# harskish/fluctus

Measured on AMD Instinct MI355X. Metric: Mrays/s (primary+shadow) at 1080p, 8 bounces, higher is better.
Workload: dtype f32; 1 GPU; kitchen-proc (procedural stand-in for Country Kitchen OBJ), 1920x1080, 8 bounces, env-map MIS under night.hdr, separate material queues; width=1920, height=1080, max_bounces=8, triangles=495648, bvh=sbvh, bvh_nodes=342315, num_tasks_per_gpu=16777216, num_tasks_whole_job=16777216, scaling_mode=weak: --num-tasks paths in flight per rank, wavefronts_per_gpu=1, fused_logic_materials=True, fused_bsdf_set=1, ext_order=2, refill_extend=8208, overlap=2, regroup=1

## Files before the change

fluctus_amd/csrc/api.hip:

```cpp
#include "flx_ctx.h"
#include <cstring>
#include <cstdlib>

thread_local std::string flxd::g_create_error;

static uint32_t localPixels(const flx_ctx *c)
{
    uint32_t npix = c->params.width * c->params.height;
    if (npix <= c->fr.rank) return 1;
    return (npix - c->fr.rank + c->fr.nranks - 1) / c->fr.nranks;
}

static int allocMoments(flx_ctx *c)
{
    freeAll(c->momAllocs);
    c->fr.moments = nullptr;
    if (!c->moments || !c->fr.localPixels) return 0;
    const size_t n = (size_t)c->fr.localPixels * 4;
    HIPCHK(c, dalloc(c, c->momAllocs, &c->fr.moments, n) ? hipErrorOutOfMemory : hipSuccess);
    HIPCHK(c, hipMemsetAsync(c->fr.moments, 0, n * 4, c->stream));
    return 0;
}
static int allocAov(flx_ctx *c)
{
    c->dn.release();
    freeAll(c->aovAllocs);
    c->fr.aovAlbedo = c->fr.aovNormal = c->fr.aovAlbedoOut = c->fr.aovNormalOut = nullptr;
    if (!c->denoiser || !c->fr.localPixels) return 0;
    const size_t n = (size_t)c->fr.localPixels * 4;
    float *buf[4] = {nullptr, nullptr, nullptr, nullptr};
    for (int i = 0; i < 4; i++) {
        HIPCHK(c, dalloc(c, c->aovAllocs, &buf[i], n) ? hipErrorOutOfMemory : hipSuccess);
        HIPCHK(c, hipMemsetAsync(buf[i], 0, n * 4, c->stream));
    }
    c->fr.aovAlbedo = buf[0]; c->fr.aovNormal = buf[1]; c->fr.aovAlbedoOut = buf[2]; c->fr.aovNormalOut = buf[3];
    return 0;
}

static int allocFrame(flx_ctx *c)
{
    uint32_t lp = localPixels(c);
    if (lp == c->fr.localPixels && c->fr.pixels) return 0;
    HIPCHK(c, hipStreamSynchronize(c->stream));
    c->releaseFrameFeatures();
    freeAll(c->frameAllocs);
    HIPCHK(c, dalloc(c, c->frameAllocs, &c->fr.pixels, (size_t)lp * 4) ? hipErrorOutOfMemory : hipSuccess);
    HIPCHK(c, dalloc(c, c->frameAllocs, &c->fr.preview, (size_t)lp * 4) ? hipErrorOutOfMemory : hipSuccess);
    HIPCHK(c, hipMemsetAsync(c->fr.pixels, 0, (size_t)lp * 16, c->stream));
    HIPCHK(c, hipMemsetAsync(c->fr.preview, 0, (size_t)lp * 16, c->stream));
    c->fr.localPixels = lp;
    if (allocMoments(c)) return 1;
    return allocAov(c);
}

static bool refill_value_ok(int v) { return v == 0 || (v > 0 && (v & 0xFF) >= 1 && (v & 0xFF) <= 64 && (v >> 8) <= 64); }

void flxd::pickSchedule(flx_ctx *c)
{
    c->overlap = c->overlapOpt >= 0 ? c->overlapOpt : 2;
    c->refillShadow = c->refillShadowOpt >= 0 ? c->refillShadowOpt : 0;
}

static int optionBuffers(flx_ctx *c, bool split, bool regen)
{
    HIPCHK(c, hipSetDevice(c->device));
    if (split && !c->splitRecA) {
        uint32_t *cnt = nullptr; uint4 *a = nullptr, *b = nullptr;
        if (dalloc(c, c->fixedAllocs, &cnt, shadow_split_count_words()) || dalloc(c, c->fixedAllocs, &a, (size_t)c->splitCapA * shadow_split_lists() * 4) ||
            dalloc(c, c->fixedAllocs, &b, (size_t)c->splitCapB * shadow_split_lists() * 4)) { c->err = "flx_set_option(shadow_split): out of device memory for the continuation records"; return 1; }
        HIPCHK(c, hipMemsetAsync(cnt, 0, (size_t)shadow_split_count_words() * 4, c->stream));
        c->splitCounts = cnt; c->splitRecA = a; c->splitRecB = b;
    }
    if (regen && !c->lookback) {
        unsigned long long *lb = nullptr;
        if (dalloc(c, c->fixedAllocs, &lb, (size_t)logic_lookback_words(c->numTasks))) { c->err = "flx_set_option(regen): out of device memory for the look-back words"; return 1; }
        HIPCHK(c, hipMemsetAsync(lb, 0, (size_t)logic_lookback_words(c->numTasks) * 8, c->stream));
        c->lookback = lb;
    }
    return 0;
}

extern "C" {

const char *flx_last_error(flx_ctx *c) { return c ? c->err.c_str() : g_create_error.c_str(); }

int flx_create(int device, uint32_t num_tasks, flx_ctx **out)
{
    *out = nullptr;
    int ndev = 0;
    hipError_t e = hipGetDeviceCount(&ndev);
    if (e != hipSuccess || ndev <= 0) { g_create_error = "flx_create: no HIP device available (libfluctus_hip.so has no CPU fallback)"; return 1; }
    if (device < 0 || device >= ndev) { g_create_error = "flx_create: bad device index"; return 1; }
    if (num_tasks == 0) { g_create_error = "flx_create: num_tasks must be > 0"; return 1; }
    flx_ctx *c = new flx_ctx();
    c->device = device; c->numTasks = num_tasks;
#ifdef FLX_LAB
    if (const char *e = getenv("FLX_REFILL_EXTEND")) { const int v = atoi(e); if (refill_value_ok(v)) c->refillExt = v; }
    if (const char *e = getenv("FLX_REFILL_SHADOW")) { const int v = atoi(e); if (v < 0 || refill_value_ok(v)) { c->refillShadowOpt = v; c->refillShadow = v < 0 ? 0 : v; } }
#endif
    auto fail = [&](const char *what, hipError_t err) { g_create_error = std::string(what) + ": " + hipGetErrorString(err); flx_destroy(c); return 1; };
    if ((e = hipSetDevice(device)) != hipSuccess) return fail("hipSetDevice", e);
#ifndef FLX_STREAM_PRIO
#define FLX_STREAM_PRIO 0
#endif
    {
        int least = 0, greatest = 0;
        (void)hipDeviceGetStreamPriorityRange(&least, &greatest);
        const int pMain = FLX_STREAM_PRIO ? greatest : 0, pSecond = FLX_STREAM_PRIO ? least : 0;
        if ((e = hipStreamCreateWithPriority(&c->stream, hipStreamNonBlocking, pMain)) != hipSuccess) return fail("hipStreamCreate", e);
        if ((e = hipStreamCreateWithPriority(&c->stream2, hipStreamNonBlocking, pSecond)) != hipSuccess) return fail("hipStreamCreate", e);
    }
    if ((e = hipEventCreateWithFlags(&c->evPreExt, hipEventDisableTiming)) != hipSuccess || (e = hipEventCreateWithFlags(&c->evShadow, hipEventDisableTiming)) != hipSuccess ||
        (e = hipEventCreateWithFlags(&c->evPostLogic, hipEventDisableTiming)) != hipSuccess) return fail("hipEventCreate", e);
    const size_t N = num_tasks;
    c->st.numTasks = num_tasks;
    for (int r = 0; r < S_NUM_REC; r++) {
        if (dalloc(c, c->fixedAllocs, &c->st.rec[r], N)) return fail("hipMalloc(state)", hipErrorOutOfMemory);
        (void)hipMemsetAsync(c->st.rec[r], 0, N * sizeof(float4), c->stream);
    }
    if (dalloc(c, c->fixedAllocs, &c->st.phase, N) || dalloc(c, c->fixedAllocs, &c->mkStats, 4)) return fail("hipMalloc(state)", hipErrorOutOfMemory);
    (void)hipMemsetAsync(c->st.phase, 0, N * 4, c->stream); (void)hipMemsetAsync(c->mkStats, 0, 16, c->stream);
    if (dalloc(c, c->fixedAllocs, &c->st.blocked, N) || dalloc(c, c->fixedAllocs, &c->st.pickProb, N) || dalloc(c, c->fixedAllocs, &c->st.firstDiffuse, N))
        return fail("hipMalloc(state)", hipErrorOutOfMemory);
    (void)hipMemsetAsync(c->st.blocked, 0, N * 4, c->stream); (void)hipMemsetAsync(c->st.pickProb, 0, N * 4, c->stream); (void)hipMemsetAsync(c->st.firstDiffuse, 0, N * 4, c->stream);
    for (int q = 0; q < FLX_NUM_QUEUES; q++) {
        if (dalloc(c, c->fixedAllocs, &c->qs.q[q], N)) return fail("hipMalloc(queue)", hipErrorOutOfMemory);
        (void)hipMemsetAsync(c->qs.q[q], 0, N * 4, c->stream);
    }
    if (dalloc(c, c->fixedAllocs, &c->qs.counters, 8) || dalloc(c, c->fixedAllocs, &c->qs.cursors, FLX_NUM_BLOCK_CURSORS * FLX_CURSOR_STRIDE)) return fail("hipMalloc(counters)", hipErrorOutOfMemory);
    (void)hipMemsetAsync(c->qs.counters, 0, 32, c->stream);
    (void)hipMemsetAsync(c->qs.cursors, 0, 4 * FLX_NUM_BLOCK_CURSORS * FLX_CURSOR_STRIDE, c->stream);
    const size_t auxStride = logic_aux_stride(num_tasks);
    const size_t queueAuxWords = logic_queue_aux_words(num_tasks);
    if (dalloc(c, c->fixedAllocs, &c->member, N) || dalloc(c, c->fixedAllocs, &c->blockCounts, (size_t)7 * auxStride) || dalloc(c, c->fixedAllocs, &c->queueAux, queueAuxWords))
        return fail("hipMalloc(logic aux)", hipErrorOutOfMemory);
    if (dalloc(c, c->fixedAllocs, &c->logicError, 1)) return fail("hipMalloc(logic error flag)", hipErrorOutOfMemory);
    (void)hipMemsetAsync(c->logicError, 0, 4, c->stream);
    (void)hipMemsetAsync(c->blockCounts, 0, (size_t)7 * auxStride * 4, c->stream);
    (void)hipMemsetAsync(c->queueAux, 0, queueAuxWords * 4, c->stream);
    { hipDeviceProp_t prop; if (hipGetDeviceProperties(&prop, device) == hipSuccess && prop.multiProcessorCount > 0) c->numCUs = prop.multiProcessorCount; }
    if (dalloc(c, c->fixedAllocs, &c->stats, FLX_NUM_TRACE_STATS)) return fail("hipMalloc(stats)", hipErrorOutOfMemory);
    (void)hipMemsetAsync(c->stats, 0, FLX_NUM_TRACE_STATS * 8, c->stream);
#ifdef FLX_LAB_RSTATS
    flxd::g_lab_rstats = c->stats;
#endif
    c->splitCapA = ((num_tasks / 2 / shadow_split_lists()) + 64u) & ~63u; c->splitCapB = ((num_tasks / 8 / shadow_split_lists()) + 64u) & ~63u;
    if (dalloc(c, c->fixedAllocs, &c->totals, 8)) return fail("hipMalloc(totals)", hipErrorOutOfMemory);
    (void)hipMemsetAsync(c->totals, 0, 64, c->stream);
    if (dalloc(c, c->fixedAllocs, &c->fr.currPixelIdx, 1)) return fail("hipMalloc(cursor)", hipErrorOutOfMemory);
    (void)hipMemsetAsync(c->fr.currPixelIdx, 0, 4, c->stream);
    c->fr.rank = 0; c->fr.nranks = 1; c->fr.localPixels = 0;
    if ((e = hipHostMalloc((void **)&c->pinned, sizeof(flx_queue_counters) * c->pinnedSlots)) != hipSuccess) return fail("hipHostMalloc", e);
    if ((e = hipHostMalloc((void **)&c->pinnedIdx, sizeof(uint32_t) * c->pinnedSlots)) != hipSuccess) return fail("hipHostMalloc", e);
    if ((e = hipHostMalloc((void **)&c->pinnedMk, 16 * c->pinnedSlots)) != hipSuccess) return fail("hipHostMalloc", e);
    {
        float4 *rgba; float2 *rec; float *pdf;
        if (dalloc(c, c->envAllocs, &rgba, 1) || dalloc(c, c->envAllocs, &rec, 1) || dalloc(c, c->envAllocs, &pdf, 1))
            return fail("hipMalloc(env)", hipErrorOutOfMemory);
        const float one = 1.0f; const float2 rec1 = make_float2(1.0f, 0.0f );
        (void)hipMemsetAsync(rgba, 0, 16, c->stream);
        (void)hipMemcpy(rec, &rec1, 8, hipMemcpyHostToDevice); (void)hipMemcpy(pdf, &one, 4, hipMemcpyHostToDevice);
        c->sc.envRGBA = rgba; c->sc.aliasRec = rec; c->sc.pdfTable = pdf; c->sc.envW = c->sc.envH = 1;
        float4 *nee; if (dalloc(c, c->envAllocs, &nee, 2)) return fail("hipMalloc(env)", hipErrorOutOfMemory);
        launch_env_nee_table(c->stream, c->sc, nee, 1u); c->sc.neeRec = nee;
    }
    if ((e = hipStreamSynchronize(c->stream)) != hipSuccess) return fail("hipStreamSynchronize", e);
    *out = c;
    return 0;
}

int flx_destroy(flx_ctx *c)
{
    if (!c) return 0;
    c->phase = PH_IDLE;
    (void)hipSetDevice(c->device);
    if (c->stream) (void)hipStreamSynchronize(c->stream);
    if (c->comm) { flx_group_destroy(c); }
    c->releaseFrameFeatures(); c->gather.release(); c->ob.release(); c->ml.releaseBuffers();
    freeAll(c->sceneAllocs); freeAll(c->spillAllocs); freeAll(c->envAllocs); freeAll(c->frameAllocs); freeAll(c->aovAllocs); freeAll(c->momAllocs); freeAll(c->fixedAllocs);
    if (c->pinned) (void)hipHostFree(c->pinned);
    if (c->pinnedIdx) (void)hipHostFree(c->pinnedIdx);
    if (c->pinnedMk) (void)hipHostFree(c->pinnedMk);
    for (auto &ev : c->events) { (void)hipEventDestroy(ev.a); (void)hipEventDestroy(ev.b); }
    for (auto e : c->eventPool) (void)hipEventDestroy(e);
    if (c->stream2) { (void)hipStreamSynchronize(c->stream2); (void)hipStreamDestroy(c->stream2); }
    if (c->evPreExt) (void)hipEventDestroy(c->evPreExt);
    if (c->evShadow) (void)hipEventDestroy(c->evShadow);
    if (c->evPostLogic) (void)hipEventDestroy(c->evPostLogic);
    if (c->stream) (void)hipStreamDestroy(c->stream);
    delete c;
    return 0;
}

uint32_t flx_num_tasks(flx_ctx *c) { return c->numTasks; }
void *flx_stream(flx_ctx *c) { (void)enter(c, CALL_PEEK); return (void *)c->stream; }

int flx_set_params(flx_ctx *c, const void *p240)
{
    ENTER(c, CALL_OBSERVE);
    NEED(c, p240, "flx_set_params: null");
    HIPCHK(c, hipSetDevice(c->device));
    const uint32_t oldW = c->params.width, oldH = c->params.height;
    memcpy(&c->params, p240, sizeof(flx_render_params));
    NEED(c, c->params.width > 0 && c->params.height > 0, "flx_set_params: zero-sized framebuffer");
    if (c->params.width != oldW || c->params.height != oldH) { c->ad.state.dropped(); c->temporal.state.imageResized(); }
    c->haveParams = true;
    return allocFrame(c);
}

int flx_set_partition(flx_ctx *c, uint32_t rank, uint32_t nranks)
{
    ENTER(c, CALL_OBSERVE);
    NEED(c, nranks >= 1 && rank < nranks, "flx_set_partition: bad rank");
    c->fr.rank = rank; c->fr.nranks = nranks;
    c->ad.state.dropped();
    c->temporal.state.partitionSet();
    return c->haveParams ? allocFrame(c) : 0;
}
uint32_t flx_local_pixels(flx_ctx *c) { return c->fr.localPixels; }

int flx_get_counters_async(flx_ctx *c, void *out32)
{
    NEED(c, out32, "flx_get_counters_async: null");
    ENTER(c, CALL_QUIET);
    HIPCHK(c, hipSetDevice(c->device));
    flushExt(c);
    if ((int)c->pending.size() >= c->pinnedSlots) { c->err = "too many outstanding counter reads; call flx_finish"; return 1; }
    int slot = c->nextSlot; c->nextSlot = (c->nextSlot + 1) % c->pinnedSlots;
    HIPCHK(c, hipMemcpyAsync(&c->pinned[slot], c->qs.counters, 32, hipMemcpyDeviceToHost, c->stream));
    c->pending.push_back({out32, slot});
    return 0;
}

int flx_finish(flx_ctx *c)
{
    ENTER(c, CALL_QUIET);
    HIPCHK(c, hipSetDevice(c->device));
    HIPCHK(c, hipStreamSynchronize(c->stream));
    if (c->regenUsed) {
        uint32_t e = 0; HIPCHK(c, hipMemcpy(&e, c->logicError, 4, hipMemcpyDeviceToHost));
        c->regenUsed = false;
        if (e) {
            HIPCHK(c, hipMemset(c->logicError, 0, 4));
            c->err = "k_logic: the in-kernel regeneration's look-back timed out (paths regenerated by that pass are invalid: reset the renderer)"; return 1;
        }
    }
    for (auto &p : c->pending) memcpy(p.user, &c->pinned[p.slot], 32);
    c->pending.clear();
    for (auto &p : c->pendingMk) memcpy(p.first, c->pinnedMk + 4 * p.second, 16);
    c->pendingMk.clear();
    for (auto &ev : c->events) {
        float ms = 0.0f;
        if (hipEventElapsedTime(&ms, ev.a, ev.b) == hipSuccess) { c->kMs[ev.kernel] += ms; c->kLaunches[ev.kernel]++; }
        c->eventPool.push_back(ev.a); c->eventPool.push_back(ev.b);
    }
    c->events.clear();
    return 0;
}

int flx_pixel_index_update(flx_ctx *c, uint32_t npix, uint32_t nnew)
{
    ENTER(c, CALL_NEUTRAL);
    NEED(c, npix > 0, "flx_pixel_index_update: zero pixels");
    HIPCHK(c, hipSetDevice(c->device));
    c->hostPixelIdx = (uint32_t)(((uint64_t)c->hostPixelIdx + nnew) % npix);
    int slot = c->nextIdxSlot; c->nextIdxSlot = (c->nextIdxSlot + 1) % c->pinnedSlots;
    c->pinnedIdx[slot] = c->hostPixelIdx;
    HIPCHK(c, hipMemcpyAsync(c->fr.currPixelIdx, &c->pinnedIdx[slot], 4, hipMemcpyHostToDevice, c->stream));
    return 0;
}
int flx_pixel_index_reset(flx_ctx *c)
{
    ENTER(c, CALL_NEUTRAL);
    HIPCHK(c, hipSetDevice(c->device));
    c->hostPixelIdx = 0;
    HIPCHK(c, hipMemsetAsync(c->fr.currPixelIdx, 0, 4, c->stream));
    return 0;
}

int flx_counter_totals(flx_ctx *c, uint64_t *out8, int reset)
{
    ENTER(c, CALL_QUIET);
    HIPCHK(c, hipSetDevice(c->device));
    HIPCHK(c, hipMemcpyAsync(out8, c->totals, 64, hipMemcpyDeviceToHost, c->stream));
    if (reset) HIPCHK(c, hipMemsetAsync(c->totals, 0, 64, c->stream));
    HIPCHK(c, hipStreamSynchronize(c->stream));
    return 0;
}

int flx_read_pixels(flx_ctx *c, int which, float *out)
{
    ENTER(c, CALL_NEUTRAL);
    NEED(c, c->fr.pixels && out, "flx_read_pixels: no framebuffer");
    HIPCHK(c, hipSetDevice(c->device));
    NEED(c, which >= 0 && which <= 7, "flx_read_pixels: which must be 0..7");
    NEED(c, which != 6 || c->dn.have, "flx_read_pixels: which = 6 is the output of flx_denoise (option \"denoiser\" on): none since the buffers were made");
    NEED(c, which != 7 || c->fr.moments, "flx_read_pixels: which = 7 (the luminance moments) needs flx_set_option(ctx, \"moments\", 1)");
    const float *src[8] = {c->fr.pixels, c->fr.preview, c->fr.aovAlbedoOut, c->fr.aovNormalOut, c->fr.aovAlbedo, c->fr.aovNormal, c->dn.out, c->fr.moments};
    NEED(c, src[which], "flx_read_pixels: the denoiser feature buffers need flx_set_option(ctx, \"denoiser\", 1)");
    HIPCHK(c, hipMemcpyAsync(out, src[which], (size_t)c->fr.localPixels * 16, hipMemcpyDeviceToHost, c->stream));
    HIPCHK(c, hipStreamSynchronize(c->stream));
    return 0;
}
int flx_write_pixels(flx_ctx *c, int which, const float *in)
{
    ENTER(c, CALL_NEUTRAL);
    NEED(c, c->fr.pixels && in, "flx_write_pixels: no framebuffer");
    HIPCHK(c, hipSetDevice(c->device));
    NEED(c, which == 0 || which == 4 || which == 5 || which == 7, "flx_write_pixels: which must be 0, 4 or 5, or 7 with option \"moments\"");
    NEED(c, which != 7 || c->fr.moments, "flx_write_pixels: which = 7 (the luminance moments) needs flx_set_option(ctx, \"moments\", 1)");
    float *dst = which == 0 ? c->fr.pixels : which == 4 ? c->fr.aovAlbedo : which == 5 ? c->fr.aovNormal : c->fr.moments;
    NEED(c, dst, "flx_write_pixels: the denoiser feature buffers need flx_set_option(ctx, \"denoiser\", 1)");
    HIPCHK(c, hipMemcpyAsync(dst, in, (size_t)c->fr.localPixels * 16, hipMemcpyHostToDevice, c->stream));
    HIPCHK(c, hipStreamSynchronize(c->stream));
    return 0;
}
int flx_copy_pixels_to_device(flx_ctx *c, void *dst)
{
    ENTER(c, CALL_OBSERVE);
    NEED(c, c->fr.pixels && dst, "flx_copy_pixels_to_device: no framebuffer");
    HIPCHK(c, hipSetDevice(c->device));
    HIPCHK(c, hipMemcpyAsync(dst, c->fr.pixels, (size_t)c->fr.localPixels * 16, hipMemcpyDeviceToDevice, c->stream));
    return 0;
}

int flx_set_option(flx_ctx *c, const char *name, int value)
{
    ENTER(c, CALL_PEEK);
    if (name && strcmp(name, "xcd_remap") == 0) { c->xcdRemap = value; return 0; }
    if (name && strcmp(name, "fuse") == 0 && (value == 0 || value == 1)) { c->fuse = value; return 0; }
    if (name && strcmp(name, "ext_order") == 0 && value >= 0 && value <= 2) { c->extOrder = value; return 0; }
    if (name && strcmp(name, "regen") == 0 && (value == 0 || value == 1)) { if (value && optionBuffers(c, false, true)) return 1; c->regenOpt = value; return 0; }
    if (name && strcmp(name, "regen_prep") == 0 && (value == 0 || value == 1)) { c->prepOpt = value; return 0; }
    if (name && strcmp(name, "regroup") == 0 && value >= -1 && value <= 1) { c->regroupOpt = value; c->regroup = value >= 0 ? value : c->regroupAuto; return 0; }
    if (name && strcmp(name, "fuse_set") == 0 && (value == 1 || value == 31)) { c->fuseSet = value; return 0; }
    if (name && strcmp(name, "overlap") == 0 && value >= -1 && value <= 2) { ENTER(c, CALL_OBSERVE); c->overlapOpt = value; pickSchedule(c); return 0; }
    if (name && strcmp(name, "shadow_tree") == 0 && (value == 2 || value == 4)) { ENTER(c, CALL_OBSERVE); c->shadowTree = value; return 0; }
    if (name && strcmp(name, "extend_tree") == 0 && (value == 2 || value == 4)) { ENTER(c, CALL_OBSERVE); c->extendTree = value; return 0; }
    if (name && strcmp(name, "denoiser") == 0 && (value == 0 || value == 1)) {
        ENTER(c, CALL_OBSERVE);
        if (c->denoiser != value) { c->denoiser = value; HIPCHK(c, hipSetDevice(c->device)); HIPCHK(c, hipStreamSynchronize(c->stream)); return allocAov(c); }
        return 0;
    }
    if (name && strcmp(name, "moments") == 0 && (value == 0 || value == 1)) {
        ENTER(c, CALL_OBSERVE);
        if (!value) c->ad.state.dropped();
        if (c->moments != value) { c->moments = value; HIPCHK(c, hipSetDevice(c->device)); HIPCHK(c, hipStreamSynchronize(c->stream)); return allocMoments(c); }
        return 0;
    }
    if (name && strcmp(name, "motion_history") == 0 && (value == 0 || value == 1)) {
        ENTER(c, CALL_OBSERVE);
        NEED(c, !value || !c->deformHistory, "flx_set_option: \"motion_history\" cannot be switched on while \"deform_history\" is on (which keeps the history across flx_objects_pose too)");
        if (!value) c->temporal.state.motionHistoryOff();
        c->motionHistory = value;
        return 0;
    }
    if (name && strcmp(name, "deform_history") == 0 && (value == 0 || value == 1)) {
        ENTER(c, CALL_OBSERVE);
        NEED(c, !value || !c->motionHistory, "flx_set_option: \"deform_history\" cannot be switched on while \"motion_history\" is on (switch that off: this option follows a pose too)");
        if (!value) c->temporal.state.deformHistoryOff();
        c->deformHistory = value;
        return 0;
    }
    if (name && strcmp(name, "mesh_lights") == 0 && (value == 0 || value == 1)) {
        ENTER(c, CALL_OBSERVE);
        c->ml.state.optionSet(value != 0);
        return meshLightsSync(c);
    }
    if (name && strcmp(name, "mesh_lights_wavefront") == 0 && (value == 0 || value == 1)) {
        ENTER(c, CALL_OBSERVE);
        c->ml.state.wavefrontSet(value != 0);
        return 0;
    }
    if (name && strcmp(name, "refill_extend") == 0 && refill_value_ok(value)) { ENTER(c, CALL_OBSERVE); c->refillExt = value; return 0; }
    if (name && strcmp(name, "refill_shadow") == 0 && (value == -1 || refill_value_ok(value))) { ENTER(c, CALL_OBSERVE); c->refillShadowOpt = value; pickSchedule(c); return 0; }
    if (name && (strcmp(name, "refill_extend") == 0 || strcmp(name, "refill_shadow") == 0)) { c->err = "flx_set_option: refill value must be 0 or refillMin (1..64) | waitMax (0..64) << 8"; return 1; }
    if (name && strcmp(name, "shadow_split") == 0 && value >= 0 && (value & 0xFF) <= 255 && (value >> 8) <= 255 && ((value & 0xFF) > 0 || value == 0)) { ENTER(c, CALL_OBSERVE); if (value && optionBuffers(c, true, false)) return 1; c->shadowSplit = value; return 0; }
    if (name && strcmp(name, "shadow_split_limit") == 0 && value >= 0) { ENTER(c, CALL_OBSERVE); c->splitLimit = (uint32_t)value; return 0; }
    if (name && strcmp(name, "eager_bump") == 0 && (value == 0 || value == 1)) { c->eagerBump = value; return 0; }
    if (name && strcmp(name, "node_layout") == 0 && (value == 0 || value == 1)) { c->nodeLayout = value; return 0; }
    c->err = std::string("flx_set_option: unknown option ") + (name ? name : "(null)");
    return 1;
}
static int phaseCode(const flx_ctx *c)
{
    return c->phase | (c->rawHits ? 8 : 0) | (c->matQueuesEmpty ? 16 : 0);
}
int flx_get_option(flx_ctx *c, const char *name, int *value)
{
    NEED(c, name && value, "flx_get_option: null");
    const struct { const char *n; int v; } tab[] = {
        {"xcd_remap", c->xcdRemap}, {"fuse", c->fuse}, {"overlap", c->overlap}, {"shadow_tree", c->shadowTree}, {"extend_tree", c->extendTree},
        {"denoiser", c->denoiser}, {"moments", c->moments}, {"motion_history", c->motionHistory}, {"deform_history", c->deformHistory},{"mesh_lights", c->ml.state.on ? 1 : 0}, {"mesh_lights_wavefront", c->ml.state.wavefront ? 1 : 0}, {"eager_bump", c->eagerBump}, {"node_layout", c->nodeLayout}, {"fuse_set", c->fuseSet}, {"ext_order", c->extOrder}, {"regen", c->regenOpt}, {"regroup", c->regroup}, {"regen_prep", c->prepOpt}, {"refill_extend", c->refillExt}, {"refill_shadow", c->refillShadow}, {"shadow_split", c->shadowSplit}, {"fused_queue_mask", (int)fused_queue_mask(fuseSetNow(c))}, {"fuse_set_now", fuseSetNow(c)}};
    for (const auto &t : tab) if (strcmp(name, t.n) == 0) { *value = t.v; return 0; }
    if (strcmp(name, "phase") == 0) { *value = phaseCode(c); return 0; }
    if (strcmp(name, "wide_far") == 0) { *value = wideFar(c); return 0; }
    c->err = std::string("flx_get_option: unknown option ") + name;
    return 1;
}

}
```

fluctus_amd/csrc/api_wavefront.hip:

```cpp
#include "flx_ctx.h"

struct Step { bool launchDeferred, commitRaw; int next; };
static Step transition(int ph, Call call)
{
    const bool deferred = ph == PH_DEFER_LOGIC || ph == PH_DEFER_LOGIC_RAYGEN;
    const bool chain = deferred || ph == PH_CHAIN || ph == PH_CHAIN_EXT;
    switch (call) {
    case CALL_LOGIC:     return {deferred, false, PH_IDLE};
    case CALL_RAYGEN:    if (ph == PH_DEFER_LOGIC) return {false, false, PH_DEFER_LOGIC_RAYGEN};
                         return {deferred, false, chain ? PH_CHAIN : PH_IDLE};
    case CALL_MATERIALS: if (deferred) return {false, false, PH_CHAIN};
                         return {false, true, chain ? PH_CHAIN : PH_IDLE};
    case CALL_EXTEND:    return {deferred, true, chain ? PH_CHAIN_EXT : PH_EXT};
    case CALL_SHADOW:    return {deferred, false, PH_IDLE};
    case CALL_QUIET:     return {deferred, false, deferred ? PH_CHAIN : ph};
    case CALL_NEUTRAL:   return {deferred, false, PH_IDLE};
    case CALL_PEEK:      return {deferred, true, deferred ? PH_CHAIN : ph};
    case CALL_OBSERVE:   return {deferred, true, PH_IDLE};
    }
    return {deferred, true, PH_IDLE};
}
void flxd::flushExt(flx_ctx *c) { if (c->qs.extPend) { launch_bump_extension(c->stream, c->qs.counters, c->qs.extPend); c->qs.extPend = 0; } }
static void flushExtIfPending(flx_ctx *c, uint32_t bits) { if (c->qs.extPend & bits) flushExt(c); }
static int runRaygen(flx_ctx *c, int appendExt = 1, bool alreadyDone = false, bool prepared = false)
{
    flushExtIfPending(c, 1u << FLX_Q_RAYGEN);
    if (!alreadyDone) { ScopedTimer t(c, FLX_K_RAYGEN); launch_raygen(c->stream, c->st, c->qs, c->fr, c->params, appendExt, prepared ? 1 : 0); }
    c->qs.extPend |= 1u << FLX_Q_RAYGEN;
    if (c->eagerBump) flushExt(c);
    LAUNCHED(c);
    return 0;
}
static int materialise(flx_ctx *c)
{
    if (!c->rawHits) return 0;
    c->rawHits = false;
    HIPCHK(c, hipSetDevice(c->device));
    launch_materialise(c->stream, c->st, c->sc, c->params, (uint32_t)c->numCUs);
    LAUNCHED(c);
    return 0;
}
static int extOrderFor(const flx_ctx *c, int fused, int raygenFirst) { return !fused ? 0 : (c->extOrder == 2 && (!raygenFirst || !c->raygenQueueEmpty)) ? 1 : c->extOrder; }
int flxd::fuseSetNow(const flx_ctx *c) { return c->params.wfSeparateQueues ? c->fuseSet : 31; }
static int runLogic(flx_ctx *c, int first, int fused, int raygenFirst)
{
    const int raw = (c->rawHits && fused != 0 && raygenFirst && !first) ? 1 : 0;
    if (!raw && materialise(c)) return 1;
    c->rawHits = false;
    flushExt(c);
#ifdef FLX_LAB_NOJOIN
    if (c->labIter >= 2) HIPCHK(c, hipStreamWaitEvent(c->stream, c->evLab[c->labIter & 1u], 0));
#endif
    const int order = extOrderFor(c, fused, raygenFirst);
    const int regen = (raw && c->regenOpt && c->lookback && logic_can_regenerate() && c->raygenQueueEmpty && c->fr.localPixels > 0 && c->numTasks <= (1u << 26)) ? 1 : 0;
    c->regenDone = regen != 0;
    if (regen) c->regenUsed = true;
    const int prep = (raw && !regen && c->prepOpt && c->raygenQueueEmpty && c->fr.localPixels > 0) ? 1 : 0;
    c->prepDone = prep != 0;
    if (++c->logicEpoch == 0u) c->logicEpoch = 1u;
    { ScopedTimer t(c, fused ? FLX_K_LOGIC_FUSED : FLX_K_LOGIC); launch_logic(c->stream, c->st, c->qs, c->sc, c->fr, c->params, c->member, c->blockCounts, c->queueAux, first, fused, raygenFirst, order, raw,
                                                                                c->lookback, c->logicEpoch, regen ? 1 : (prep ? 2 : 0), order == 2 ? 0 : 1, c->logicError, c->regroup,
                                                                                c->queueParity ^= 1u, (uint32_t)c->numCUs,
                                                                                (!fused && c->ml.state.litWavefront()) ? &c->ml.t : nullptr); }
    LAUNCHED(c);
    c->matQueuesEmpty = false; c->raygenQueueEmpty = false;
    if (c->overlap == 2) HIPCHK(c, hipEventRecord(c->evPostLogic, c->stream));
    return 0;
}
static uint32_t materialBits(const flx_ctx *c)
{
    return c->params.wfSeparateQueues ? ((1u << FLX_Q_DIFFUSE) | (1u << FLX_Q_GLOSSY) | (1u << FLX_Q_GGX_REFL) | (1u << FLX_Q_GGX_REFR) | (1u << FLX_Q_DELTA)) : (1u << FLX_Q_DIFFUSE);
}
int flxd::enter(flx_ctx *c, Call call)
{
    const Step st = transition(c->phase, call);
    if (st.launchDeferred) {
        const bool withRaygen = c->phase == PH_DEFER_LOGIC_RAYGEN;
        c->phase = PH_CHAIN;
        HIPCHK(c, hipSetDevice(c->device));
        if (runLogic(c, c->pendFirst, 0, 0)) return 1;
        if (withRaygen && runRaygen(c)) return 1;
    }
    if (st.commitRaw && materialise(c)) return 1;
    c->phase = st.next;
    return 0;
}

extern "C" {

int flx_wf_reset(flx_ctx *c) { READY(c, CALL_OBSERVE); flushExt(c); c->temporal.state.accumulationReset(); c->raygenQueueEmpty = false;  { ScopedTimer t(c, FLX_K_RESET); launch_reset(c->stream, c->st, c->qs, c->fr, c->params); } LAUNCHED(c); return 0; }
int flx_wf_raygen(flx_ctx *c)
{
    if (c->phase == PH_DEFER_LOGIC) { ENTER(c, CALL_RAYGEN); return 0; }
    READY(c, CALL_RAYGEN);
    return runRaygen(c);
}
int flx_wf_extend(flx_ctx *c)
{
    READY(c, CALL_EXTEND);
    const bool chainIntact = c->phase == PH_CHAIN_EXT;
    if (c->overlap && !(c->overlap == 2 && chainIntact)) HIPCHK(c, hipEventRecord(c->evPreExt, c->stream));
    if (c->profile == 1 || c->profile == 2) { if (c->spanStart) c->eventPool.push_back(c->spanStart); c->spanStart = getEvent(c); (void)hipEventRecord(c->spanStart, c->stream); }
    {
        ScopedTimer t(c, FLX_K_EXTEND);
        if (c->extendTree == 4 && c->wideOK && c->refillExt > 0 && !c->statsOn) {
            uint32_t *cur = c->qs.cursors;
            if (c->cursorDirty[0]) HIPCHK(c, hipMemsetAsync(cur, 0, 4 * 8 * FLX_CURSOR_STRIDE, c->stream));
            launch_extend4r(c->stream, c->st, c->qs, c->sc, c->params, c->spill, (uint32_t)c->numCUs, c->refillExt, cur);
            c->cursorDirty[0] = true; c->rawHits = true;
        }
        else if (c->extendTree == 4 && c->wideOK) launch_extend4(c->stream, c->st, c->qs, c->sc, c->params, c->spill, c->statsOn ? c->stats : nullptr);
        else launch_extend(c->stream, c->st, c->qs, c->sc, c->params, c->spill, c->statsOn ? c->stats : nullptr, c->xcdRemap);
    }
    LAUNCHED(c);
    return 0;
}
int flx_wf_shadow(flx_ctx *c)
{
    const bool overlapped = (c->phase == PH_CHAIN_EXT || c->phase == PH_EXT) && c->overlap != 0;
    const bool early = c->phase == PH_CHAIN_EXT && c->overlap == 2;
    READY(c, CALL_SHADOW);
    hipStream_t s = c->stream;
    if (overlapped) { s = c->stream2; HIPCHK(c, hipStreamWaitEvent(s, early ? c->evPostLogic : c->evPreExt, 0)); }
    hipEvent_t earlyStart = nullptr;
    if ((c->profile == 1 || c->profile == 2) && early) { earlyStart = getEvent(c); (void)hipEventRecord(earlyStart, s); }
    {
        ScopedTimer t(c, FLX_K_SHADOW, s);
        uint32_t *spill = overlapped ? c->spill2 : c->spill;
        if (c->shadowTree == 4 && c->wideOK && c->refillShadow > 0 && !c->statsOn) {
            uint32_t *cur = c->qs.cursors + 8 * FLX_CURSOR_STRIDE;
            if (c->cursorDirty[1]) HIPCHK(c, hipMemsetAsync(cur, 0, 4 * 8 * FLX_CURSOR_STRIDE, s));
            launch_shadow4r(s, c->st, c->qs, c->sc, c->params, spill, (uint32_t)c->numCUs, c->refillShadow, cur);
            c->cursorDirty[1] = true;
        }
#ifdef FLX_LAB_NOJOIN
        else if (c->shadowTree == 4 && c->wideOK && overlapped) {
            if (!c->labCounters) HIPCHK(c, hipMalloc(&c->labCounters, 2 * 32));
            Queues q2 = c->qs; q2.counters = c->labCounters + 8 * (c->labIter & 1u);
            HIPCHK(c, hipMemcpyAsync(q2.counters, c->qs.counters, 32, hipMemcpyDeviceToDevice, s));
            launch_shadow4(s, c->st, q2, c->sc, c->params, spill, nullptr);
        }
#endif
        else if (c->shadowTree == 4 && c->wideOK && c->shadowSplit > 0 && !c->statsOn)
            launch_shadow4_split(s, c->st, c->qs, c->sc, c->params, spill, c->splitCounts, c->splitParity++, c->splitRecA, c->splitCapA, c->splitRecB, c->splitCapB, c->shadowSplit & 0xFF, c->shadowSplit >> 8, c->splitLimit);
        else if (c->shadowTree == 4 && c->wideOK) launch_shadow4(s, c->st, c->qs, c->sc, c->params, spill, c->statsOn ? c->stats : nullptr);
        else launch_shadow(s, c->st, c->qs, c->sc, c->params, spill, c->statsOn ? c->stats : nullptr, c->xcdRemap);
    }
    LAUNCHED(c);
#ifdef FLX_LAB_NOJOIN
    if (overlapped) {
        if (!c->evLab[0]) { HIPCHK(c, hipEventCreateWithFlags(&c->evLab[0], hipEventDisableTiming)); HIPCHK(c, hipEventCreateWithFlags(&c->evLab[1], hipEventDisableTiming)); }
        HIPCHK(c, hipEventRecord(c->evLab[c->labIter & 1u], s)); c->labIter++;
        return 0;
    }
#endif
    if (overlapped) { HIPCHK(c, hipEventRecord(c->evShadow, s)); HIPCHK(c, hipStreamWaitEvent(c->stream, c->evShadow, 0)); }
    if ((c->profile == 1 || c->profile == 2) && overlapped && c->spanStart) {
        hipEvent_t b = getEvent(c); (void)hipEventRecord(b, c->stream);
        if (earlyStart) { c->eventPool.push_back(c->spanStart); c->spanStart = earlyStart; earlyStart = nullptr; }
        c->events.push_back({FLX_K_TRACE_SPAN, c->spanStart, b}); c->spanStart = nullptr;
    }
    if (earlyStart) c->eventPool.push_back(earlyStart);
    return 0;
}
int flx_wf_logic(flx_ctx *c, int first)
{
    READY(c, CALL_LOGIC);
    const uint32_t allMat = (1u << FLX_Q_DIFFUSE) | (1u << FLX_Q_GLOSSY) | (1u << FLX_Q_GGX_REFL) | (1u << FLX_Q_GGX_REFR) | (1u << FLX_Q_DELTA);
    const bool fusable = c->params.wfSeparateQueues || fused_queue_mask(fuseSetNow(c)) == allMat;
    if (c->fuse && c->matQueuesEmpty && fusable && !c->ml.state.litWavefront()) { c->phase = PH_DEFER_LOGIC; c->pendFirst = first; }
    else { if (runLogic(c, first, 0, 0)) return 1; c->phase = PH_CHAIN; }
    return 0;
}
int flx_wf_materials(flx_ctx *c)
{
    const int before = c->phase;
    if (before == PH_DEFER_LOGIC || before == PH_DEFER_LOGIC_RAYGEN) {
        const bool withRaygen = before == PH_DEFER_LOGIC_RAYGEN;
        ENTER(c, CALL_MATERIALS);
        NEED(c, c->haveParams && c->sc.bnodes, "set params and upload a scene first");
        HIPCHK(c, hipSetDevice(c->device));
        const int fuseNow = fuseSetNow(c);
        const int order = extOrderFor(c, fuseNow, withRaygen);
        if (runLogic(c, c->pendFirst, fuseNow, withRaygen)) return 1;
        if (withRaygen && runRaygen(c, order == 2 ? 0 : 1, c->regenDone, c->prepDone)) return 1;
        c->regenDone = false; c->prepDone = false;
        { ScopedTimer t(c, FLX_K_MATERIALS); launch_materials_after_fused(c->stream, c->st, c->qs, c->sc, fused_queue_mask(fuseNow), order); }
        LAUNCHED(c);
        c->qs.extPend |= materialBits(c);
        if (c->eagerBump) flushExt(c);
        return 0;
    }
    READY(c, CALL_MATERIALS);
    const uint32_t bits = materialBits(c);
    flushExtIfPending(c, bits);
    { ScopedTimer t(c, FLX_K_MATERIALS); launch_materials(c->stream, c->st, c->qs, c->sc, c->params.wfSeparateQueues); }
    c->qs.extPend |= bits;
    if (c->eagerBump) flushExt(c);
    LAUNCHED(c); return 0;
}
int flx_clear_queues(flx_ctx *c)
{
    ENTER(c, CALL_NEUTRAL);
    c->qs.extPend = 0; c->matQueuesEmpty = true; c->raygenQueueEmpty = true;
    HIPCHK(c, hipSetDevice(c->device));
    HIPCHK(c, hipMemsetAsync(c->qs.counters, 0, 32, c->stream));
    if (c->cursorDirty[0] || c->cursorDirty[1]) {
        HIPCHK(c, hipMemsetAsync(c->qs.cursors, 0, 4 * FLX_NUM_BLOCK_CURSORS * FLX_CURSOR_STRIDE, c->stream));
        c->cursorDirty[0] = c->cursorDirty[1] = false;
    }
    return 0;
}

int flx_end_iteration_async(flx_ctx *c)
{
    READY(c, CALL_NEUTRAL);
    launch_end_iteration(c->stream, c->qs.counters, c->totals, c->fr.currPixelIdx, c->fr.localPixels, c->qs.extPend, c->qs.cursors);
    c->cursorDirty[0] = c->cursorDirty[1] = false;
    c->qs.extPend = 0;
    c->matQueuesEmpty = true; c->raygenQueueEmpty = true;
    LAUNCHED(c);
    return 0;
}

}
```

fluctus_amd/csrc/flx_ctx.h:

```cpp
#pragma once
#include "flx_launch.h"
#include "flx_feature_state.h"
#include "../../include/fluctus_hip.h"
#include <string>
#include <vector>
#include <utility>
#include <rccl/rccl.h>

using namespace flxd;

namespace flxd {
struct PendingCounters { void *user; int slot; };
struct PendingEvent { int kernel; hipEvent_t a, b; };
inline void freeAll(std::vector<void *> &v) { for (void *p : v) (void)hipFree(p); v.clear(); }

enum Phase { PH_IDLE = 0, PH_DEFER_LOGIC = 1, PH_DEFER_LOGIC_RAYGEN = 2, PH_CHAIN = 3, PH_CHAIN_EXT = 4, PH_EXT = 5 };
enum Call {
    CALL_LOGIC, CALL_RAYGEN, CALL_MATERIALS, CALL_EXTEND, CALL_SHADOW,
    CALL_QUIET,
    CALL_NEUTRAL,
    CALL_PEEK,
    CALL_OBSERVE
};
}

struct flx_ctx {
    int device = 0;
    hipStream_t stream = nullptr;
    hipStream_t stream2 = nullptr;
    hipEvent_t evPreExt = nullptr, evShadow = nullptr, evPostLogic = nullptr;
#ifdef FLX_LAB_NOJOIN
    hipEvent_t evLab[2] = {nullptr, nullptr}; uint32_t labIter = 0; uint32_t *labCounters = nullptr;
#endif
    int phase = 0;
    int overlap = 2;
    int overlapOpt = -1;
    uint32_t *spill2 = nullptr;
    int fuse = 1;
    int extOrder = 0;
    int fuseSet = 1;
    int regroup = 0, regroupAuto = 0, regroupOpt = -1;
    int pendFirst = 0;
    bool matQueuesEmpty = false;
    bool raygenQueueEmpty = false;
    uint32_t numTasks = 0;
    std::string err;
    State st {};
    Queues qs {};
    Scene sc {};
    Frame fr {};
    flx_render_params params {};
    bool haveParams = false;
    uint32_t hostPixelIdx = 0;
    uint8_t *member = nullptr; uint32_t *blockCounts = nullptr;
    uint32_t *queueAux = nullptr; uint32_t queueParity = 0;
    unsigned long long *lookback = nullptr; uint32_t logicEpoch = 0; uint32_t *logicError = nullptr; int regenOpt = 0; bool regenDone = false; bool regenUsed = false; int prepOpt = 1; bool prepDone = false;
    uint32_t *spill = nullptr;
    unsigned long long *stats = nullptr;
    unsigned long long *totals = nullptr;
    uint32_t *mkStats = nullptr;
    uint32_t *pinnedMk = nullptr; std::vector<std::pair<void *, int>> pendingMk; int nextMkSlot = 0;
    bool statsOn = false;
    int xcdRemap = 0;
    int shadowTree = 4, extendTree = 4;
    int refillExt = 16 | (32 << 8), refillShadow = 0;
    int refillShadowOpt = -1;
    int shadowSplit = 0;
    uint32_t splitParity = 0;
    uint32_t splitLimit = 0;
    uint32_t *splitCounts = nullptr; uint4 *splitRecA = nullptr, *splitRecB = nullptr; uint32_t splitCapA = 0, splitCapB = 0;
    bool rawHits = false;
    bool cursorDirty[2] = {false, false};

    uint32_t wideInfo[8] = {0, 0, 0, 0, 0, 0, 0, 0};
    RefitTables rf;
    bool wideOK = false;
    uint32_t spillLevels = 0;
    int eagerBump = 0;
    int denoiser = 0;
    std::vector<void *> aovAllocs;
    struct Denoise {
        std::vector<void *> allocs;
        float4 *e[2] = {nullptr, nullptr}, *g = nullptr; float2 *g2 = nullptr; float *out = nullptr;
        bool have = false;
        void release() { freeAll(allocs); *this = Denoise(); }
    } dn;
    int moments = 0;
    std::vector<void *> momAllocs;
    struct Temporal {
        std::vector<void *> allocs;
        float4 *gb[2] = {nullptr, nullptr}, *hist = nullptr, *histMomBuf = nullptr; uint32_t *objPlane[2] = {nullptr, nullptr};
        float2 *baryPlane[2] = {nullptr, nullptr};
        float4 *mark = nullptr, *markMomBuf = nullptr, *rcRec = nullptr; float *lambda = nullptr;
        TemporalState state;
        void release() { freeAll(allocs); *this = Temporal(); }
    } temporal;
    int motionHistory = 0;
    int deformHistory = 0;
    struct Adaptive {
        std::vector<void *> allocs;
        uint8_t *flags = nullptr; uint32_t *scratch = nullptr, *list = nullptr, *countDev = nullptr;
        ActiveListState state;
        void release() { freeAll(allocs); *this = Adaptive(); }
    } ad;
    void releaseFrameFeatures() { dn.release(); temporal.release(); ad.release(); }
    struct Objects {
        std::vector<void *> allocs;
        ObjectTables t;
        std::vector<uint32_t> counts;
        bool have = false;
        PoseState pose;
        uint32_t *objectOfTri = nullptr; float4 *motion = nullptr, *motionPinned = nullptr;
        void release() { freeAll(allocs); if (motionPinned) (void)hipHostFree(motionPinned); *this = Objects(); }
    } ob;
    struct MeshLight {
        std::vector<void *> allocs;
        std::vector<uint32_t> list;
        MeshLights t;
        MeshLightState state;
        void releaseBuffers() { freeAll(allocs); t = MeshLights(); }
    } ml;
    int nodeLayout = 1;
    int numCUs = 256;
    ncclComm_t comm = nullptr;
    bool commShared = false;
    struct Gather {
        std::vector<void *> allocs;
        float *stage = nullptr, *full = nullptr; size_t stageFloats = 0, fullFloats = 0;
        void release() { freeAll(allocs); *this = Gather(); }
    } gather;
    std::vector<void *> sceneAllocs, envAllocs, frameAllocs, fixedAllocs, spillAllocs;
    flx_queue_counters *pinned = nullptr; int pinnedSlots = 64, nextSlot = 0;
    uint32_t *pinnedIdx = nullptr; int nextIdxSlot = 0;
    std::vector<PendingCounters> pending;
    int profile = 0;
    hipEvent_t spanStart = nullptr;
    std::vector<PendingEvent> events;
    std::vector<hipEvent_t> eventPool;
    double kMs[FLX_K_COUNT] = {0}; uint64_t kLaunches[FLX_K_COUNT] = {0};
};

#define HIPCHK(c, expr) do { hipError_t e_ = (expr); if (e_ != hipSuccess) { (c)->err = std::string(#expr) + ": " + hipGetErrorString(e_); return 1; } } while (0)
#define NEED(c, cond, msg) do { if (!(cond)) { (c)->err = msg; return 1; } } while (0)
#define ENTER(c, call) do { if (enter(c, call)) return 1; } while (0)
#define READY(c, call) do { ENTER(c, call); NEED(c, (c)->haveParams, "set params first (flx_set_params)"); NEED(c, (c)->sc.bnodes, "upload a scene first (flx_upload_scene)"); HIPCHK(c, hipSetDevice((c)->device)); } while (0)
#define LAUNCHED(c) HIPCHK(c, hipGetLastError())

namespace flxd {
template <class T> int dalloc(flx_ctx *c, std::vector<void *> &own, T **p, size_t count)
{
    void *d = nullptr;
    HIPCHK(c, hipMalloc(&d, (count ? count : 1) * sizeof(T)));
    own.push_back(d);
    *p = (T *)d;
    return 0;
}

inline hipEvent_t getEvent(flx_ctx *c)
{
    if (!c->eventPool.empty()) { hipEvent_t e = c->eventPool.back(); c->eventPool.pop_back(); return e; }
    hipEvent_t e; (void)hipEventCreate(&e); return e;
}
struct ScopedTimer {
    flx_ctx *c; int k; hipStream_t s; hipEvent_t a = nullptr, b = nullptr;
    bool on;
    ScopedTimer(flx_ctx *c_, int k_, hipStream_t s_ = nullptr) : c(c_), k(k_), s(s_ ? s_ : c_->stream)
    {
        on = c->profile == 1 || (c->profile == 2 && (k == FLX_K_EXTEND || k == FLX_K_SHADOW)) || (c->profile == 3 && k == FLX_K_EXTEND) ||
             (c->profile == 4 && (k == FLX_K_EXTEND || k == FLX_K_SHADOW || k == FLX_K_LOGIC || k == FLX_K_LOGIC_FUSED));
        if (on) { a = getEvent(c); b = getEvent(c); (void)hipEventRecord(a, s); }
    }
    ~ScopedTimer() { if (on) { (void)hipEventRecord(b, s); c->events.push_back({k, a, b}); } }
};

extern thread_local std::string g_create_error;
int enter(flx_ctx *c, Call call);
void flushExt(flx_ctx *c);
int fuseSetNow(const flx_ctx *c);
float wideClampFor(float maxAbsCoord);
int motionTables(flx_ctx *c);
int meshLightsSync(flx_ctx *c);
int wideFar(const flx_ctx *c);
void pickSchedule(flx_ctx *c);
}
```

fluctus_amd/csrc/flx_device.h:

```cpp
#pragma once
#include <hip/hip_runtime.h>
#include <stdint.h>
#include "../../include/fluctus_wire.h"
#include "../../include/flx_math.h"

namespace flxd {

using namespace flx;

enum { S_ORIG = 0, S_DIR, S_HITP, S_HITN, S_HITUV, S_THR, S_EI, S_SHO, S_SHD, S_LBSDF, S_LEMIT, S_LT, S_NUM_REC };

struct State {
    float4 *rec[S_NUM_REC];
    __host__ __device__ __forceinline__ float4 *at(int r, uint32_t gid) const { return rec[r] + (size_t)gid; }
    uint32_t *blocked;
    float *pickProb;
    uint32_t *firstDiffuse;
    uint32_t *phase;
    uint32_t numTasks;
};

#define FLX_NUM_BLOCK_CURSORS 16
#define FLX_CURSOR_STRIDE 64

struct Queues {
    uint32_t *q[FLX_NUM_QUEUES];
    uint32_t *counters;
    uint32_t *cursors;
    uint32_t extPend;
};

#define FLX_LEAF_BIT 0x80000000u

struct BNode {
    float lmin[3], lmax[3];
    float rmin[3], rmax[3];
    uint32_t left, right;
    uint32_t pad[2];
};

struct TriRec {
    float4 a;
    float4 b;
    float4 c;
};

struct ShadeRec {
    float4 a;
    float4 b;
    float4 c;
    float4 d;
};

struct Scene {
    const BNode *bnodes;
    const TriRec *trirecs;
    const ShadeRec *shade;
    const flx_triangle *tris;
    const flx_material *materials;
    const flx_texdesc *texdesc;
    const uint8_t *texdata;
    uint32_t rootRef;
    const void *wnodes;
    const float4 *wleaf;
    uint32_t wrootRef;
    float wideClamp;
    const float4 *envRGBA;
    const float *pdfTable;
    const float2 *aliasRec;
    const float4 *neeRec;
    int envW, envH;
};

struct Frame {
    float *pixels;
    float *preview;
    float *aovAlbedo, *aovNormal, *aovAlbedoOut, *aovNormalOut;
    float *moments;
    uint32_t *currPixelIdx;
    uint32_t rank, nranks;
    uint32_t localPixels;
};

__device__ __forceinline__ f3 ld3(const float4 &v) { return mk3(v.x, v.y, v.z); }
__device__ __forceinline__ float4 mk4(f3 v, float w) { return make_float4(v.x, v.y, v.z, w); }
__device__ __forceinline__ float4 mk4u(f3 v, uint32_t w) { return make_float4(v.x, v.y, v.z, __uint_as_float(w)); }
__device__ __forceinline__ f3 V(const flx_vec3 &v) { return mk3(v.x, v.y, v.z); }
__device__ __forceinline__ f3 camera_space_normal(const flx_render_params &p, f3 N)
{
    const f3 r1 = V(p.camera.right), r2 = V(p.camera.up), r3 = V(p.camera.dir) * -1.0f;
    return mk3(dot(r1, N), dot(r2, N), dot(r3, N));
}

#ifndef FLX_NT
#define FLX_NT 3
#endif
typedef float flx_v4f __attribute__((ext_vector_type(4)));
__device__ __forceinline__ float4 rd4(const float4 *p)
{
#if FLX_NT & 1
    flx_v4f v = __builtin_nontemporal_load(reinterpret_cast<const flx_v4f *>(p));
    return make_float4(v.x, v.y, v.z, v.w);
#else
    return *p;
#endif
}
__device__ __forceinline__ float4 rd4t(const float4 *p) { return *p; }
__device__ __forceinline__ void wr4(float4 *p, float4 v)
{
#if FLX_NT & 2
    flx_v4f t; t.x = v.x; t.y = v.y; t.z = v.z; t.w = v.w;
    __builtin_nontemporal_store(t, reinterpret_cast<flx_v4f *>(p));
#else
    *p = v;
#endif
}

__device__ __forceinline__ void wr4t(float4 *p, float4 v) { *p = v; }

#define FLX_FRESH 0x80000000u

__device__ __forceinline__ uint32_t lane_id() { return __builtin_amdgcn_mbcnt_hi(~0u, __builtin_amdgcn_mbcnt_lo(~0u, 0u)); }
__device__ __forceinline__ uint32_t mbcnt(uint64_t mask)
{
    return __builtin_amdgcn_mbcnt_hi((uint32_t)(mask >> 32), __builtin_amdgcn_mbcnt_lo((uint32_t)mask, 0u));
}


__device__ __forceinline__ uint32_t ext_len(const Queues &qs)
{
    uint32_t n = qs.counters[FLX_Q_EXTENSION];
    if (qs.extPend) for (int q = 0; q < FLX_NUM_QUEUES; q++) if (qs.extPend & (1u << q)) n += qs.counters[q];
    return n;
}

}
```

fluctus_amd/csrc/flx_launch.h:

```cpp
#pragma once
#include "flx_device.h"
#include <vector>

namespace flx { struct ad_params; struct rp_view; struct rp_params; struct rc_params; }

namespace flxd {
struct RefitTables {
    uint32_t ntris = 0, nidx = 0, nmat = 0, nwtri = 0, nwleaf = 0;
    uint32_t *blevel = nullptr, *wlevel = nullptr;
    std::vector<uint32_t> blevelStart, wlevelStart;
    uint32_t *wtriOff = nullptr, *wleafOff = nullptr;
    float4 *wexact = nullptr;
    uint32_t *valid = nullptr;
    void *stage = nullptr;
    double *costSlab = nullptr;
    uint32_t *triStamp = nullptr, *bStamp = nullptr, *wStamp = nullptr, *lStamp = nullptr;
    size_t stampWords = 0;
    uint32_t epoch = 0;
    uint32_t *stageIdx = nullptr;
    float4 *snapPos = nullptr; uint8_t *movedFlags = nullptr;
};
void launch_refit_validate(hipStream_t, const void *, const uint32_t *, uint32_t, const Scene &, const RefitTables &, uint32_t *);
void launch_refit(hipStream_t, const void *, const uint32_t *, uint32_t, const Scene &, const RefitTables &);
struct ObjectTables {
    uint32_t nobjects = 0, members = 0;
    uint32_t *memberTri = nullptr, *memberObj = nullptr;
    float4 *rest = nullptr;
    uint32_t *stamp = nullptr, *slot = nullptr;
    uint32_t *ids = nullptr; float4 *xforms = nullptr;
    float4 *out = nullptr; uint32_t *outIdx = nullptr;
    uint32_t *blockCounts = nullptr, *total = nullptr;
    uint32_t epoch = 0;
};
struct MeshLights {
    uint32_t n = 0;
    uint32_t *tri = nullptr;
    float *w = nullptr, *cdf = nullptr, *pick = nullptr;
    double *local = nullptr;
    double *runSum = nullptr, *off = nullptr; uint32_t *runLast = nullptr;
    double *total = nullptr;
    uint32_t *hdr = nullptr;
};
__device__ __forceinline__ void ml_vertices(const Scene &sc, uint32_t tri, f3 *p0, f3 *p1, f3 *p2)
{
    const float4 *t = reinterpret_cast<const float4 *>(sc.tris + tri);
    *p0 = ld3(t[0]); *p1 = ld3(t[3]); *p2 = ld3(t[6]);
}
__device__ __forceinline__ int ml_material(const Scene &sc, uint32_t tri) { return sc.tris[tri].matId; }
template <bool MESH> struct MeshArg { static constexpr bool on = false; __device__ MeshLights get() const { return MeshLights(); } };
template <> struct MeshArg<true> { static constexpr bool on = true; MeshLights t; __device__ MeshLights get() const { return t; } };
uint32_t mesh_light_runs(uint32_t n);
void launch_mesh_light_build(hipStream_t, const Scene &, const MeshLights &);
void launch_mesh_light_probe(hipStream_t, const Scene &, const MeshLights &, const float *, uint32_t, uint32_t *, float *);
uint32_t pose_blocks(uint32_t members);
void launch_pose(hipStream_t, const ObjectTables &, uint32_t count);
void launch_object_of_triangle(hipStream_t, const ObjectTables &, uint32_t *objectOfTri);
void launch_block_scan(hipStream_t, uint32_t *blockCounts, uint32_t nb, uint32_t *total);
size_t tree_cost_slab_doubles(const RefitTables &);
double *launch_tree_cost(hipStream_t, const Scene &, const RefitTables &, double *);
void launch_extend(hipStream_t, const State &, const Queues &, const Scene &, const flx_render_params &, uint32_t *, unsigned long long *, int);
void launch_shadow(hipStream_t, const State &, const Queues &, const Scene &, const flx_render_params &, uint32_t *, unsigned long long *, int);
void launch_extend4(hipStream_t, const State &, const Queues &, const Scene &, const flx_render_params &, uint32_t *, unsigned long long *);
void launch_shadow4(hipStream_t, const State &, const Queues &, const Scene &, const flx_render_params &, uint32_t *, unsigned long long *);
void launch_shadow4_split(hipStream_t, const State &, const Queues &, const Scene &, const flx_render_params &, uint32_t *, uint32_t *, uint32_t, uint4 *, uint32_t, uint4 *, uint32_t, int, int, uint32_t);
uint32_t shadow_split_lists(); uint32_t shadow_split_count_words();
void launch_extend4r(hipStream_t, const State &, const Queues &, const Scene &, const flx_render_params &, uint32_t *, uint32_t, int, uint32_t *);
void launch_shadow4r(hipStream_t, const State &, const Queues &, const Scene &, const flx_render_params &, uint32_t *, uint32_t, int, uint32_t *);
void launch_logic(hipStream_t, const State &, const Queues &, const Scene &, const Frame &, const flx_render_params &, uint8_t *, uint32_t *, uint32_t *, int, int, int, int, int,
                  unsigned long long *, uint32_t, int, int, uint32_t *, int, uint32_t, uint32_t, const MeshLights *);
void launch_env_nee_table(hipStream_t, const Scene &, float4 *, uint32_t);
int logic_can_regenerate();
uint32_t logic_lookback_words(uint32_t numTasks);
void launch_materialise(hipStream_t, const State &, const Scene &, const flx_render_params &, uint32_t);
void launch_materials(hipStream_t, const State &, const Queues &, const Scene &, uint32_t);
void launch_materials_after_fused(hipStream_t, const State &, const Queues &, const Scene &, uint32_t, int);
uint32_t fused_queue_mask(int);
uint32_t logic_aux_stride(uint32_t);
uint32_t logic_queue_aux_words(uint32_t);
void launch_reset(hipStream_t, const State &, const Queues &, const Frame &, const flx_render_params &);
void launch_raygen(hipStream_t, const State &, const Queues &, const Frame &, const flx_render_params &, int, int);
void launch_postprocess(hipStream_t, const Frame &, const flx_render_params &);
void launch_state_export(hipStream_t, const State &, float *, float);
void launch_state_import(hipStream_t, const State &, const float *);
void launch_math_probe(hipStream_t, int, const float *, const float *, uint32_t, uint32_t *);
void launch_mk_reset(hipStream_t, const State &, const Frame &, const flx_render_params &);
void launch_mk_raygen(hipStream_t, const State &, const flx_render_params &, const uint32_t *, uint32_t);
void launch_mk_next_vertex(hipStream_t, const State &, const Scene &, const Frame &, const flx_render_params &, uint32_t *, uint32_t *, const uint32_t *, uint32_t, const MeshLights *);
void launch_mk_sample_bsdf(hipStream_t, const State &, const Scene &, const Frame &, const flx_render_params &, uint32_t *, uint32_t *, const uint32_t *, uint32_t, const MeshLights *);
void launch_mk_splat(hipStream_t, const State &, const Frame &, const flx_render_params &, uint32_t *, int, const uint32_t *, uint32_t);
uint32_t adaptive_blocks(uint32_t);
void launch_adaptive_update(hipStream_t, const float4 *, int, int, const ad_params &, uint8_t *, uint32_t *, uint32_t *, uint32_t *);
void launch_end_iteration(hipStream_t, uint32_t *, unsigned long long *, uint32_t *, uint32_t, uint32_t, uint32_t *);
void launch_bump_extension(hipStream_t, uint32_t *, uint32_t);
void launch_deinterleave(hipStream_t, const float *, float *, uint32_t, uint32_t, uint32_t);
struct DnGuided; struct DnVg;
template <class F> void launch_denoise(hipStream_t, const Frame &, float4 *, float4 *, float4 *, float2 *, float *, int, int, int, float, float, float,
                                       float, const flx_render_params &);
void launch_gbuffer(hipStream_t, const Scene &, const flx_render_params &, uint32_t *, uint32_t, int, float4 *, uint32_t, uint32_t *, const uint32_t *, float2 *);
void launch_reproject(hipStream_t, const rp_view &, const rp_params &, const float4 *, const float4 *, const float4 *, const float4 *, float4 *, float4 *);
void launch_reproject_motion(hipStream_t, const rp_view &, const rp_params &, const float4 *, const float4 *, const float4 *, const float4 *, float4 *, float4 *,
                             const uint32_t *, const uint32_t *, const float4 *, uint32_t);
void launch_snapshot_positions(hipStream_t, const Scene &, uint32_t, float4 *);
void launch_moved_flags(hipStream_t, const Scene &, uint32_t, const float4 *, uint8_t *);
void launch_reproject_deform(hipStream_t, const rp_view &, const rp_params &, const float4 *, const float4 *, const float4 *, const float4 *, float4 *, float4 *,
                             const float2 *, const float2 *, const Scene &, uint32_t, const float4 *, const uint8_t *);
void launch_rectify(hipStream_t, const rc_params &, float, int, int, const float4 *, float4 *, float4 *, float4 *, float4 *, float4 *, float *);
#ifdef FLX_LAB_RSTATS
extern unsigned long long *g_lab_rstats;
#endif
}
```

fluctus_amd/csrc/flx_trace.h:

```cpp
#pragma once
#include "flx_device.h"

namespace flxd {

#ifndef TRACE_BLOCK
#define TRACE_BLOCK 64
#endif
#ifndef LDS_LEVELS
#define LDS_LEVELS 16
#endif
#ifndef TRACE_MIN_WAVES
#define TRACE_MIN_WAVES 1
#endif
#ifndef SHADOW_MIN_WAVES
#define SHADOW_MIN_WAVES 1
#endif

struct TraceAux {
    uint32_t *spill;
    uint32_t totalThreads;
    unsigned long long *stats;
};

__device__ __forceinline__ bool slab(const float *bmin, const float *bmax, f3 orig, f3 dinv, float tMaxPrev, float *tnear)
{
    f3 tmp = (mk3(bmin[0], bmin[1], bmin[2]) - orig) * dinv;
    f3 tmaxv = (mk3(bmax[0], bmax[1], bmax[2]) - orig) * dinv;
    f3 tminv = min3(tmp, tmaxv);
    tmaxv = max3(tmp, tmaxv);
    float tmin = fmaxf_(fmaxf_(tminv.x, tminv.y), tminv.z);
    float tmax = fminf_(fminf_(tmaxv.x, tmaxv.y), tmaxv.z);
    *tnear = tmin;
    if (tmax < 0.0f) return false;
    if (tmin > tmax) return false;
    return tmin < tMaxPrev;
}

__device__ __forceinline__ bool moller_trumbore(f3 orig, f3 dir, f3 p0, f3 p1, f3 p2, float *tret, float *uret, float *vret)
{
    f3 s1 = p1 - p0;
    f3 s2 = p2 - p0;
    f3 pvec = cross(dir, s2);
    float det = dot(s1, pvec);
    if (absf(det) < 1e-12f) return false;
    float iDet = 1.0f / det;
    f3 tvec = orig - p0;
    float u = dot(tvec, pvec) * iDet;
    if (u < 0.0f || u > 1.0f) return false;
    f3 qvec = cross(tvec, s1);
    float v = dot(dir, qvec) * iDet;
    if (v < 0.0f || u + v > 1.0f) return false;
    float t = dot(s2, qvec) * iDet;
    if (t < 0.0f) return false;
    *tret = t; *uret = u; *vret = v;
    return true;
}

__device__ __forceinline__ bool light_quad(const flx_arealight &L, f3 orig, f3 dir, float *t)
{
    if (dot(dir, V(L.N)) > 0.0f) return false;
    f3 pos = V(L.pos), right = V(L.right), up = V(L.up);
    f3 tl = pos + L.size.x * right + L.size.y * up;
    f3 tr = pos - L.size.x * right + L.size.y * up;
    f3 bl = pos + L.size.x * right - L.size.y * up;
    f3 br = pos - L.size.x * right - L.size.y * up;
    bool hit = false;
    float tt, u, v;
    if (moller_trumbore(orig, dir, tl, bl, br, &tt, &u, &v) && !(tt > *t)) { *t = tt; hit = true; }
    if (moller_trumbore(orig, dir, tl, br, tr, &tt, &u, &v) && !(tt > *t)) { *t = tt; hit = true; }
    return hit;
}

struct HitVals { f3 P, N; float tu, tv, t; int tri, matId; uint32_t flags; };

template <bool LIGHT_QUAD = true>
__device__ __forceinline__ HitVals hit_values(const Scene &sc, const flx_render_params &p, f3 orig, f3 dir, float t, float u, float v, int tri)
{
    HitVals h;
    h.P = mk3(0.0f); h.N = mk3(0.0f);
    h.tu = 0.0f; h.tv = 0.0f;
    h.matId = -1;
    h.flags = 0;
    if (tri >= 0) {
        const float4 *sp = reinterpret_cast<const float4 *>(sc.shade + tri);
        float4 a = sp[0], b = sp[1], c = sp[2], d = sp[3];
        h.P = orig + t * dir;
        h.N = normalize(bary(u, v, ld3(a), ld3(b), ld3(c)));
        f3 uv = bary(u, v, mk3(a.w, b.w, 0.0f), mk3(c.w, d.x, 0.0f), mk3(d.y, d.z, 0.0f));
        h.tu = uv.x; h.tv = uv.y;
        h.matId = __float_as_int(d.w);
    }
    if (LIGHT_QUAD && p.sampleImpl && p.useAreaLight) {
        if (light_quad(p.areaLight, orig, dir, &t)) {
            h.flags = 1u;
            h.P = orig + t * dir;
            h.N = V(p.areaLight.N);
            tri = 0; h.matId = 0;
        }
    }
    h.t = t; h.tri = tri;
    return h;
}

__device__ __forceinline__ uint32_t hit_keep_flags(float pathLenBits, uint32_t oldHitNw)
{
    const bool first = (__float_as_uint(pathLenBits) & ~FLX_FRESH) == 0u && (__float_as_uint(pathLenBits) & FLX_FRESH) != 0u;
    return first ? 0u : (oldHitNw & 2u);
}

template <bool LIGHT_QUAD = true>
__device__ __forceinline__ void commit_hit(const State &st, const Scene &sc, const flx_render_params &p, uint32_t gid, f3 orig, f3 dir, float pathLenBits,
                                           float t, float u, float v, int tri, uint32_t &flags, int &matId)
{
    const HitVals h = hit_values<LIGHT_QUAD>(sc, p, orig, dir, t, u, v, tri);
    flags = h.flags; matId = h.matId;
    wr4(st.at(S_DIR, gid), mk4u(dir, __float_as_uint(pathLenBits) + 1u));
    wr4(st.at(S_HITP, gid), mk4(h.P, h.t));
    const uint32_t keep = hit_keep_flags(pathLenBits, __float_as_uint(reinterpret_cast<const float *>(st.at(S_HITN, gid))[3]));
    wr4(st.at(S_HITN, gid), mk4u(h.N, h.flags | keep));
    wr4(st.at(S_HITUV, gid), make_float4(h.tu, h.tv, __int_as_float(h.tri), __int_as_float(h.matId)));
}

#define FLX_RAW       0x40000000u
#define FLX_RAW_TRI   0x3FFFFFFFu
__device__ __forceinline__ bool hit_is_raw(uint32_t z) { return (z & 0xC0000000u) == FLX_RAW; }
__device__ __forceinline__ HitVals hit_values_raw(const Scene &sc, const flx_render_params &p, f3 orig, f3 dir, float4 raw)
{
    return hit_values<true>(sc, p, orig, dir, raw.w, raw.x, raw.y, (int)(__float_as_uint(raw.z) & FLX_RAW_TRI) - 1);
}

struct Stack {
    uint32_t *lds;
    uint32_t *spill;
    uint32_t stride;
    __device__ __forceinline__ void push(int level, uint32_t v)
    {
        if (level < LDS_LEVELS) lds[level * TRACE_BLOCK] = v;
        else spill[(size_t)(level - LDS_LEVELS) * stride] = v;
    }
    __device__ __forceinline__ uint32_t pop(int level)
    {
        return level < LDS_LEVELS ? lds[level * TRACE_BLOCK] : spill[(size_t)(level - LDS_LEVELS) * stride];
    }
};


__device__ __forceinline__ uint32_t xcd_remap(uint32_t b, uint32_t nblocks, int enable)
{
    if (!enable) return b;
    uint32_t per = nblocks >> 3;
    if (per == 0 || b >= (per << 3)) return b;
    return (b & 7u) * per + (b >> 3);
}

#define FLX_RAY_DONE 0xFFFFFFFFu

template <bool ANY_HIT, bool STATS>
__device__ __forceinline__ bool traverse(const Scene &sc, Stack &stk, f3 orig, f3 dir, float &tbest, float &ubest, float &vbest,
                                         int &tribest, uint32_t &nInner, uint32_t &nTri, unsigned long long *wstats = nullptr)
{
#define FLX_WAVE_TICK(k) do { if (STATS && wstats) { const uint64_t m_ = __ballot(true); \
        if (lane_id() == (uint32_t)__ffsll((long long)m_) - 1u) atomicAdd(&wstats[k], 1ull); } } while (0)
    const f3 dinv = mk3(1.0f / dir.x, 1.0f / dir.y, 1.0f / dir.z);
    int sp = 0;
    uint32_t cur = sc.rootRef;
    for (;;) {
        FLX_WAVE_TICK(0);
        while (!(cur & FLX_LEAF_BIT)) {
            FLX_WAVE_TICK(1);
            const float4 *np = reinterpret_cast<const float4 *>(sc.bnodes + cur);
            const float4 n0 = np[0], n1 = np[1], n2 = np[2], n3 = np[3];
            const float lmin[3] = {n0.x, n0.y, n0.z}, lmax[3] = {n0.w, n1.x, n1.y};
            const float rmin[3] = {n1.z, n1.w, n2.x}, rmax[3] = {n2.y, n2.z, n2.w};
            const uint32_t left = __float_as_uint(n3.x), right = __float_as_uint(n3.y);
            if (STATS) nInner++;
            float lnear, rnear;
            const bool lh = slab(lmin, lmax, orig, dinv, tbest, &lnear);
            const bool rh = slab(rmin, rmax, orig, dinv, tbest, &rnear);
            if (lh && rh) {
                const bool goRight = rnear < lnear;
                stk.push(sp++, goRight ? left : right);
                cur = goRight ? right : left;
            } else if (lh || rh) {
                cur = lh ? left : right;
            } else {
                cur = (sp == 0) ? FLX_RAY_DONE : stk.pop(sp - 1);
                sp = (sp == 0) ? 0 : sp - 1;
            }
        }
        if (cur == FLX_RAY_DONE) break;
        {
            const uint32_t slot = cur & ~FLX_LEAF_BIT;
            const float4 *tp = reinterpret_cast<const float4 *>(sc.trirecs + slot);
            float4 a = tp[0], b = tp[1], c = tp[2];
            const int count = __float_as_int(b.w);
            FLX_WAVE_TICK(2);
            for (int k = 0;;) {
                FLX_WAVE_TICK(3);
                if (STATS) nTri++;
                float t, u, v;
                if (moller_trumbore(orig, dir, ld3(a), ld3(b), ld3(c), &t, &u, &v) && t > 0.0f && t < tbest) {
                    if (ANY_HIT) return true;
                    tbest = t; ubest = u; vbest = v; tribest = __float_as_int(a.w);
                }
                if (++k >= count) break;
                tp += 3;
                a = tp[0]; b = tp[1]; c = tp[2];
            }
        }
        if (sp == 0) break;
        cur = stk.pop(--sp);
    }
    return false;
#undef FLX_WAVE_TICK
}


}
```

fluctus_amd/csrc/logic.hip:

```cpp
#include "flx_bsdf.h"
#include "flx_trace.h"
#include "flx_denoise.h"
#include "flx_launch.h"
#include "flx_splat.h"
#include "flx_light.h"
#include "flx_queue_build.h"

namespace flxd {

#ifndef LOGIC_BLOCK
#define LOGIC_BLOCK 256
#endif
__host__ __device__ constexpr bool fuse_inlines_list(int fuse, uint32_t ml)
{
    return ml == 1u ? (fuse & USE_DIFFUSE) != 0 : ml == 2u ? (fuse & USE_GLOSSY) != 0 : ml == 3u ? (fuse & USE_GGX_REFL) != 0
         : ml == 4u ? (fuse & USE_GGX_REFR) != 0 : ml == 5u ? (fuse & USE_DELTA) != 0 : false;
}
#define NUM_LISTS 7

#ifndef LOGIC_FULL_STORES
#define LOGIC_FULL_STORES 1
#endif
#ifndef LOGIC_REGROUP
#define LOGIC_REGROUP 1
#endif
#ifndef LOGIC_LAZY_HITN
#define LOGIC_LAZY_HITN 1
#endif
#ifndef LOGIC_REGROUP_MIN_BLOCKS
#define LOGIC_REGROUP_MIN_BLOCKS 5
#endif

struct LogicAux {
    uint8_t *member;
    uint32_t *blockCounts;
    uint32_t *segTotals;
    uint32_t *snapshot;
    uint32_t numBlocks;
    uint32_t numSegs;
    uint32_t stride;
    unsigned long long *lookback;
    uint32_t epoch;
    uint32_t regen;
    uint32_t appendExt;
    uint32_t *error;
};

#define LB_VALUE(x) ((uint32_t)((x) & 0x3FFFFFFull))
#define LB_FLAG(x) ((uint32_t)(((x) >> 26) & 3ull))
#define LB_EPOCH(x) ((uint32_t)((x) >> 28))
#define LB_PACK(e, f, v) (((unsigned long long)(e) << 28) | ((unsigned long long)(f) << 26) | (unsigned long long)(v))
__device__ __forceinline__ uint32_t wave_sum7(uint32_t v, bool take)
{
    uint32_t s = 0u;
    #pragma unroll
    for (int b = 0; b < 7; b++) s += (uint32_t)__popcll(__ballot(take && ((v >> b) & 1u))) << b;
    return s;
}
__device__ __forceinline__ uint32_t lookback_exclusive(const LogicAux &aux, uint32_t wave, uint32_t count)
{
    const uint32_t lane = lane_id();
    const uint32_t win = (uint32_t)__popcll(__ballot(true));
    unsigned long long *st = aux.lookback;
    if (lane == 0u) __hip_atomic_store(st + wave, LB_PACK(aux.epoch, wave == 0u ? 2u : 1u, count), __ATOMIC_RELAXED, __HIP_MEMORY_SCOPE_AGENT);
    if (wave == 0u) return 0u;
    uint32_t sum = 0u;
    long long j = (long long)wave - 1;
    for (uint32_t spins = 0;;) {
        const long long idx = j - (long long)lane;
        unsigned long long v = LB_PACK(aux.epoch, 2u, 0u);
        if (idx >= 0) v = __hip_atomic_load(st + idx, __ATOMIC_RELAXED, __HIP_MEMORY_SCOPE_AGENT);
        const bool ok = LB_EPOCH(v) == aux.epoch && LB_FLAG(v) != 0u;
        const uint64_t b2 = __ballot(ok && LB_FLAG(v) == 2u), bad = __ballot(!ok);
        const uint32_t first2 = b2 ? (uint32_t)__ffsll((long long)b2) - 1u : win;
        const uint64_t need = first2 >= 64u ? ~0ull : ((1ull << first2) | ((1ull << first2) - 1ull));
        if (bad & need) {
            if (++spins > (1u << 22)) { if (lane == 0u) *aux.error = 1u; break; }
            __builtin_amdgcn_s_sleep(2);
            continue;
        }
        sum += wave_sum7(LB_VALUE(v), lane < first2);
        if (b2) { sum += (uint32_t)__shfl((int)LB_VALUE(v), (int)first2, 64); break; }
        j -= (long long)win;
    }
    if (lane == 0u) __hip_atomic_store(st + wave, LB_PACK(aux.epoch, 2u, sum + count), __ATOMIC_RELAXED, __HIP_MEMORY_SCOPE_AGENT);
    return sum;
}

static_assert(LOGIC_BLOCK == flxqb::QB_BLOCK && NUM_LISTS == flxqb::QB_LISTS, "flx_queue_build.h counts in k_logic's blocks and lists");
__host__ __device__ constexpr uint32_t list_counter(uint32_t l) { return l == 0u ? (uint32_t)FLX_Q_RAYGEN : l + 1u; }
static_assert(list_counter(1) == FLX_Q_SHADOW && list_counter(2) == FLX_Q_DIFFUSE && list_counter(6) == FLX_Q_DELTA, "queue numbering");

__device__ __forceinline__ uint32_t material_list(int type, uint32_t separate)
{
    if (!separate) return 1u;
    switch (type) {
    case FLX_BXDF_DIFFUSE: return 1u;
    case FLX_BXDF_GLOSSY: return 2u;
    case FLX_BXDF_GGX_ROUGH_REFLECTION: return 3u;
    case FLX_BXDF_GGX_ROUGH_DIELECTRIC: return 4u;
    case FLX_BXDF_IDEAL_REFLECTION:
    case FLX_BXDF_IDEAL_DIELECTRIC: return 5u;
    default: return 0u;
    }
}

#ifndef LOGIC_MIN_BLOCKS
#define LOGIC_MIN_BLOCKS 0
#endif
template <int FUSE, bool RAW = false, bool REGROUP = false, bool MESH = false>
__global__ __launch_bounds__(LOGIC_BLOCK, (REGROUP ? LOGIC_REGROUP_MIN_BLOCKS : LOGIC_MIN_BLOCKS) > 0 ? (REGROUP ? LOGIC_REGROUP_MIN_BLOCKS : LOGIC_MIN_BLOCKS) : 1) void k_logic(State st, Scene sc, Frame fr, flx_render_params p, LogicAux aux, Queues qs, uint32_t firstIteration, MeshArg<MESH> meshArg)
{
    const MeshLights mesh = meshArg.get();
    auto kinds = [&]() { return light_kind_probs(p.useEnvMap, p.useAreaLight, MESH && lamps_pickable(mesh)); };
    const uint32_t gid = blockIdx.x * LOGIC_BLOCK + threadIdx.x;
    uint32_t maxId = st.numTasks;
    if (firstIteration) { uint32_t npix = p.width * p.height; maxId = npix < maxId ? npix : maxId; }
    uint32_t member = 0u;
    __shared__ uint32_t s_item[REGROUP ? 20 : 1][LOGIC_BLOCK];
    __shared__ uint32_t s_tc[5][LOGIC_BLOCK / 64];

    if (gid < maxId) {
        const float4 thr = rd4(st.at(S_THR, gid));
        const float4 d4 = rd4(st.at(S_DIR, gid));
        const float4 o4 = rd4(st.at(S_ORIG, gid));
        const float4 huv = rd4(st.at(S_HITUV, gid));
        float4 hn = make_float4(0.0f, 0.0f, 0.0f, 0.0f);
        if (!(RAW && LOGIC_LAZY_HITN != 0 && hit_is_raw(__float_as_uint(huv.z)))) hn = rd4(st.at(S_HITN, gid));
        const float4 ei4 = rd4(st.at(S_EI, gid));
        uint32_t seed = __float_as_uint(thr.w);
        const uint32_t pixIdx = __float_as_uint(ei4.w) & ~FLX_FRESH;
        float eiw = ei4.w;
        const f3 rayOrig = ld3(o4), rayDir = ld3(d4);
        const float lastPdfW = o4.w;
        f3 T = ld3(thr);
        f3 Ei = ld3(ei4);
        f3 hitN = ld3(hn);
        uint32_t hflags = __float_as_uint(hn.w);
        int hitI = __float_as_int(huv.z), hitMat = __float_as_int(huv.w);
        f2 hitUV = mk2(huv.x, huv.y);
        uint32_t lenBits = __float_as_uint(d4.w);
        bool isRaw = false; f3 rawP = mk3(0.0f); float rawT = 0.0f;
        if (RAW && hit_is_raw(__float_as_uint(huv.z))) {
            isRaw = true;
            const HitVals h = hit_values_raw(sc, p, rayOrig, rayDir, huv);
            hflags = h.flags | hit_keep_flags(d4.w, hflags);
            hitN = h.N; hitI = h.tri; hitMat = h.matId; hitUV = mk2(h.tu, h.tv); rawP = h.P; rawT = h.t;
            lenBits += 1u;
        }
        const uint32_t len = lenBits & ~FLX_FRESH;
        const bool fresh = (lenBits & FLX_FRESH) != 0u;
        if (fresh && len == 0u && !isRaw) { hitI = -1; hitMat = -1; hitN = mk3(0.0f); hflags = 0u; hitUV = mk2(0.0f, 0.0f); }
        bool Tdirty = false;

        bool terminate = (len >= p.maxBounces + 1u);
        const bool meshCut = MESH && terminate && !p.useRoulette;
        if (terminate && p.useRoulette) {
            float contProb = clampf(luminance(T), 0.01f, 0.5f);
            terminate = (rand01(&seed) > contProb);
            T = T / contProb;
            Tdirty = true;
        }
        if (is_zero(T) || lastPdfW == 0.0f) terminate = true;

        if (hitI < 0 && !terminate) {
            float weight = 1.0f;
            const bool lastSpecular = fresh || __float_as_uint(rd4(st.at(S_LT, gid)).w) != 0u;
            f3 bg = mk3(0.0f);
            if (p.useEnvMap && (len == 1u || p.sampleImpl)) bg = eval_env_dir(sc, rayDir) * p.envMapStrength;
            if (p.sampleImpl && p.sampleExpl && p.useEnvMap && len > 1u && !lastSpecular) {
                float lightPickProb = st.pickProb[gid];
                float directPdfW = env_map_pdf(sc, rayDir);
                weight = mis_implicit_env_reference(lastPdfW, lightPickProb, directPdfW);
                if (MESH) { const KindProbs k = kinds(); if (k.lamps) weight = mis_implicit(lastPdfW, directPdfW, k.env); }
            }
            Ei = Ei + weight * T * bg;
            terminate = true;
        } else if (p.useAreaLight && (hflags & 1u) && !terminate) {
            float misWeight = 1.0f;
            const bool lastSpecular = fresh || __float_as_uint(rd4(st.at(S_LT, gid)).w) != 0u;
            const f3 hitP = (RAW && isRaw) ? rawP : ld3(rd4(st.at(S_HITP, gid)));
            if (p.sampleExpl && len > 1u && !lastSpecular) {
                const float directPdfW = quad_pdf_w(p.areaLight, length(hitP - rayOrig), dot(normalize(-rayDir), hitN));
                misWeight = mis_implicit(lastPdfW, directPdfW, st.pickProb[gid]);
            }
            Ei = Ei + T * misWeight * V(p.areaLight.E);
            terminate = true;
        } else if (MESH && hitI >= 0 && !(hflags & 1u) && (!terminate || (meshCut && !is_zero(T) && lastPdfW != 0.0f))) {
            f3 Ke; float misWeight;
            if (lamp_implicit(sc, p, mesh, hitI, hitMat, len, rayOrig, rayDir, lastPdfW,
                              [&]() { return fresh || __float_as_uint(rd4(st.at(S_LT, gid)).w) != 0u; },
                              [&]() { return (RAW && isRaw) ? rawP : ld3(rd4(st.at(S_HITP, gid))); },
                              [&]() { return kinds().lamp; },
                              &Ke, &misWeight))
                Ei = Ei + T * misWeight * Ke;
        }

        const uint32_t blockedOld = st.blocked[gid];
        if (blockedOld == 0u) {
            float4 le = rd4(st.at(S_LEMIT, gid));
            float4 lb = rd4(st.at(S_LBSDF, gid));
            const float4 lt = rd4(st.at(S_LT, gid));
            float directPdfW = rd4(st.at(S_SHD, gid)).w;
            if (fresh) lb = make_float4(0.0f, 0.0f, 0.0f, 0.0f);
            if ((__float_as_uint(ei4.w) & FLX_FRESH) != 0u) { le = make_float4(0.0f, 0.0f, 0.0f, 0.0f); directPdfW = 0.0f; }
            const float lightPickProb = st.pickProb[gid];
            const float cosTh = le.w, bsdfPdfW = lb.w;
            Ei = Ei + nee_contribution(ld3(lb), ld3(lt), ld3(le), cosTh, directPdfW, lightPickProb, bsdfPdfW, p.sampleImpl != 0u);
        }

        constexpr bool FULL = LOGIC_FULL_STORES != 0 && RAW && FUSE != 0;
        uint32_t regenRank = 0u, regenLocal = 0u;
        const bool regen = FULL && aux.regen == 1u;
        const bool prep = FULL && aux.regen == 2u;
        if (regen) {
            const uint64_t tb = __ballot(terminate);
            regenRank = lookback_exclusive(aux, gid >> 6, (uint32_t)__popcll(tb)) + mbcnt(tb);
            regenLocal = (*fr.currPixelIdx + regenRank) % fr.localPixels;
        }
        flx_material mat;
        bool backface = false, haveL = false, neeBlocked = false, inlined = false;
        f3 hitP = rawP, orig = mk3(0.0f), Lnee = mk3(0.0f), neeLi = mk3(0.0f);
        float hitT = rawT, neeLen = 0.0f, neePdf = 0.0f, neeCos = 0.0f, neePick = 0.0f;
        uint32_t ml = 0u;
        auto splat = [&]() {
#ifndef FLX_LAB_LOGIC_NOSPLAT
            const bool add = terminate && len > 0u;
            wave_add4(fr.pixels, add, pixIdx, Ei.x, Ei.y, Ei.z, 1.0f, 0xFu);
            if (fr.moments) {
                const float l = flx_lum(Ei);
                wave_add4(fr.moments, add, pixIdx, l, l * l, 0.0f, 1.0f, 0xBu);
            }
#endif
        };
        if (!FULL) splat();
        if (terminate) {
            if (!FULL) {
                wr4(st.at(S_EI, gid), mk4(Ei, ei4.w));
                wr4(st.at(S_THR, gid), mk4u(T, seed));
                if (RAW && isRaw) wr4(st.at(S_HITUV, gid), make_float4(hitUV.x, hitUV.y, __int_as_float(hitI), __int_as_float(hitMat)));
            }
            member = 1u;
        } else {
            mat = sc.materials[hitMat];
            hitN = tangent_space_normal(sc, hitN, hitUV, hitI, mat.map_N);
            backface = dot(hitN, rayDir) > 0.0f;
            if (backface) hitN = hitN * -1.0f;
            if (!(RAW && isRaw)) { const float4 hp = rd4(st.at(S_HITP, gid)); hitP = ld3(hp); hitT = hp.w; }
            if (!FULL && RAW && isRaw) {
                if (FUSE == USE_ALL) {
                    wr4t(st.at(S_HITP, gid), mk4(rawP, rawT));
                    wr4t(st.at(S_HITUV, gid), make_float4(hitUV.x, hitUV.y, __int_as_float(hitI), __int_as_float(hitMat)));
                } else {
                    wr4(st.at(S_HITP, gid), mk4(rawP, rawT));
                    wr4(st.at(S_HITUV, gid), make_float4(hitUV.x, hitUV.y, __int_as_float(hitI), __int_as_float(hitMat)));
                }
            }
            orig = hitP - 1e-3f * rayDir;
            if (!FULL) wr4(st.at(S_HITN, gid), mk4u(hitN, (hflags & 1u) | (backface ? 2u : 0u)));

            if (p.sampleExpl && !FLX_BXDF_IS_SINGULAR(mat.type)) {
                const KindProbs kp = kinds();
                const float envMapProb = kp.env;
                const float kindDraw = rand01(&seed);
                const bool useEnvMap = kindDraw < envMapProb;
                const bool useAreaLight = !useEnvMap && p.useAreaLight && (!kp.lamps || kindDraw < kp.envOrQuad);
                const bool useMesh = kp.lamps && !useEnvMap && !useAreaLight;
                if (useEnvMap && p.useEnvMap) {
                    f3 L; float directPdfW = 0.0f;
#ifdef FLX_LAB_LOGIC_NONEE
                    { const float r = rand01(&seed); L = mk3(r - 0.5f, 0.7f, 0.3f - r); directPdfW = 0.1f + r; }
                    const float lenL = 2.0f * p.worldRadius;
                    L = normalize(L);
                    const float cosTh = fmaxf_(0.0f, dot(L, hitN));
                    const f3 envMapLi = mk3(directPdfW, cosTh, 0.5f) * p.envMapStrength;
#else
                    const int uvInd = sample_env_index(sc, rand01(&seed));
                    const float4 n0 = sc.neeRec[2 * (size_t)uvInd], n1 = sc.neeRec[2 * (size_t)uvInd + 1];
                    L = ld3(n0); directPdfW = n0.w;
                    const float lenL = 2.0f * p.worldRadius;
                    const float cosTh = fmaxf_(0.0f, dot(L, hitN));
                    const f3 envMapLi = ld3(n1) * p.envMapStrength;
#endif
                    neeLen = lenL; neePdf = directPdfW; neeLi = envMapLi; neeCos = cosTh; neePick = envMapProb;
                    haveL = true; Lnee = L;
                }
                if (useAreaLight) {
                    const LightSample ls = quad_sample(p.areaLight, orig, &seed, 0.995f);
                    if (ls.cosLight > 0.0f) {
                        neeLen = ls.rayLen; neePdf = ls.pdfW(); neeLi = V(p.areaLight.E); neeCos = fmaxf_(0.0f, dot(ls.L, hitN)); neePick = kp.quad;
                        haveL = true; Lnee = ls.L;
                    } else {
                        neeBlocked = true;
                    }
                }
                if (MESH && useMesh) {
                    uint32_t ltri;
                    const LightSample ls = lamp_sample(sc, mesh, orig, &seed, &ltri);
                    if (ls.cosLight > 0.0f) {
                        neeLen = ls.rayLen; neePdf = ls.pdfW(); neeLi = V(sc.materials[ml_material(sc, ltri)].Ke); neeCos = fmaxf_(0.0f, dot(ls.L, hitN)); neePick = kp.lamp;
                        haveL = true; Lnee = ls.L;
                    } else {
                        neeBlocked = true;
                    }
                }
                if (haveL) {
                    eiw = __uint_as_float(pixIdx);
                    member |= 2u;
                    if (!FULL) {
                        wr4(st.at(S_SHO, gid), mk4(orig, neeLen));
                        wr4(st.at(S_SHD, gid), mk4(Lnee, neePdf));
                        wr4(st.at(S_LEMIT, gid), mk4(neeLi, neeCos));
                        st.pickProb[gid] = neePick;
                    }
                }
                if (!FULL && neeBlocked) st.blocked[gid] = 1u;
            }
            if (!FULL) wr4(st.at(S_EI, gid), mk4(Ei, eiw));
            (void)Tdirty;
            ml = material_list(mat.type, p.wfSeparateQueues);
            member |= ml << 2;
            inlined = FUSE != 0 && fuse_inlines_list(FUSE, ml);
        }
        if (fr.aovNormal) {
            const bool addN = !terminate && len == 1u;
            f3 n = mk3(0.0f);
            if (addN) n = camera_space_normal(p, hitN);
            wave_add4(fr.aovNormal, addN, pixIdx, n.x, n.y, n.z, 1.0f, 0xFu);
            bool addA = false;
            f3 albedo = mk3(0.0f);
            if (!terminate) {
                const flx_material m = FUSE == USE_ALL ? sc.materials[hitMat] : mat;
                if (!FLX_BXDF_IS_SINGULAR(m.type) && !st.firstDiffuse[gid]) {
                    st.firstDiffuse[gid] = 1u;
                    albedo = mat_float3(sc, V(m.Kd), hitUV, m.map_Kd);
                    addA = true;
                }
            }
            wave_add4(fr.aovAlbedo, addA, pixIdx, albedo.x, albedo.y, albedo.z, 1.0f, 0xFu);
        }

        f3 Lold = mk3(0.0f);
        if (FULL) {
            float4 sho = mk4(orig, neeLen), shd = mk4(Lnee, neePdf), le = mk4(neeLi, neeCos);
            float pick = neePick;
#ifdef FLX_LAB_LOGIC_NOOLD
            if (!haveL && !terminate) {
#else
            if (!haveL) {
#endif
                sho = rd4(st.at(S_SHO, gid)); shd = rd4(st.at(S_SHD, gid));
                if (!terminate) { le = rd4(st.at(S_LEMIT, gid)); pick = st.pickProb[gid]; } else pick = 1.0f;
                Lold = ld3(shd);
            }
            const float4 hp4 = mk4(hitP, hitT), huv4 = make_float4(hitUV.x, hitUV.y, __int_as_float(hitI), __int_as_float(hitMat));
            if (FUSE == USE_ALL) { wr4t(st.at(S_HITP, gid), hp4); wr4t(st.at(S_HITUV, gid), huv4); }
            else { wr4(st.at(S_HITP, gid), hp4); wr4(st.at(S_HITUV, gid), huv4); }
            wr4(st.at(S_HITN, gid), mk4u(hitN, (hflags & 1u) | (backface ? 2u : 0u)));
            wr4(st.at(S_SHO, gid), sho);
            wr4(st.at(S_SHD, gid), shd);
            wr4(st.at(S_LEMIT, gid), le);
            st.pickProb[gid] = pick;
            wr4(st.at(S_EI, gid), (regen && terminate) ? mk4u(mk3(0.0f), FLX_FRESH | regenLocal) : mk4(Ei, eiw));
        }

        MatStep o;
        o.bsdfNEE = mk3(0.0f); o.bsdfPdfW = 0.0f; o.singular = 0u; o.newT = T; o.orig = mk3(0.0f); o.pdfW = 0.0f; o.newDir = mk3(0.0f);
        bool regrouped = false;
        if constexpr (REGROUP) {
            regrouped = true;
            const bool work = !terminate && inlined;
            const uint32_t wv = threadIdx.x >> 6;
            uint32_t cls = 4u;
            if (work) { const uint32_t c_ = material_list(mat.type, 1u); cls = c_ ? c_ - 1u : 4u; }
            uint64_t bt[5];
            #pragma unroll
            for (int t = 0; t < 5; t++) bt[t] = __ballot(work && cls == (uint32_t)t);
            if ((threadIdx.x & 63u) == 0u) { for (int t = 0; t < 5; t++) s_tc[t][wv] = (uint32_t)__popcll(bt[t]); }
            __syncthreads();
            uint32_t slot = 0u, total = 0u;
            #pragma unroll
            for (int t = 0; t < 5; t++) {
                uint32_t before = 0u, all = 0u;
                for (uint32_t w = 0; w < LOGIC_BLOCK / 64; w++) { const uint32_t n_ = s_tc[t][w]; all += n_; if (w < wv) before += n_; }
                if (cls == (uint32_t)t) slot = total + before + mbcnt(bt[t]);
                total += all;
            }
            if (work) {
                const f3 L = haveL ? Lnee : Lold;
                s_item[0][slot] = __float_as_uint(hitP.x); s_item[1][slot] = __float_as_uint(hitP.y); s_item[2][slot] = __float_as_uint(hitP.z);
                s_item[3][slot] = __float_as_uint(hitN.x); s_item[4][slot] = __float_as_uint(hitN.y); s_item[5][slot] = __float_as_uint(hitN.z);
                s_item[6][slot] = __float_as_uint(hitUV.x); s_item[7][slot] = __float_as_uint(hitUV.y);
                s_item[8][slot] = (uint32_t)hitMat; s_item[9][slot] = backface ? 1u : 0u;
                s_item[10][slot] = __float_as_uint(rayDir.x); s_item[11][slot] = __float_as_uint(rayDir.y); s_item[12][slot] = __float_as_uint(rayDir.z);
                s_item[13][slot] = __float_as_uint(L.x); s_item[14][slot] = __float_as_uint(L.y); s_item[15][slot] = __float_as_uint(L.z);
                s_item[16][slot] = __float_as_uint(T.x); s_item[17][slot] = __float_as_uint(T.y); s_item[18][slot] = __float_as_uint(T.z);
                s_item[19][slot] = seed;
            }
            __syncthreads();
            const uint32_t k = threadIdx.x;
            if (k < total) {
                SurfHit h;
                h.P = mk3(__uint_as_float(s_item[0][k]), __uint_as_float(s_item[1][k]), __uint_as_float(s_item[2][k]));
                h.N = mk3(__uint_as_float(s_item[3][k]), __uint_as_float(s_item[4][k]), __uint_as_float(s_item[5][k]));
                h.uv = mk2(__uint_as_float(s_item[6][k]), __uint_as_float(s_item[7][k]));
                const int mid = (int)s_item[8][k]; const bool bf = s_item[9][k] != 0u;
                const f3 dIn = mk3(__uint_as_float(s_item[10][k]), __uint_as_float(s_item[11][k]), __uint_as_float(s_item[12][k]));
                const f3 Lk = mk3(__uint_as_float(s_item[13][k]), __uint_as_float(s_item[14][k]), __uint_as_float(s_item[15][k]));
                const f3 Tk = mk3(__uint_as_float(s_item[16][k]), __uint_as_float(s_item[17][k]), __uint_as_float(s_item[18][k]));
                uint32_t sk = s_item[19][k];
                const MatStep r_ = material_step<FUSE>(sc, h, sc.materials[mid], bf, dIn, Lk, Tk, &sk);
                s_item[0][k] = __float_as_uint(r_.bsdfNEE.x); s_item[1][k] = __float_as_uint(r_.bsdfNEE.y); s_item[2][k] = __float_as_uint(r_.bsdfNEE.z);
                s_item[3][k] = __float_as_uint(r_.bsdfPdfW); s_item[4][k] = r_.singular;
                s_item[5][k] = __float_as_uint(r_.newT.x); s_item[6][k] = __float_as_uint(r_.newT.y); s_item[7][k] = __float_as_uint(r_.newT.z);
                s_item[8][k] = __float_as_uint(r_.orig.x); s_item[9][k] = __float_as_uint(r_.orig.y); s_item[10][k] = __float_as_uint(r_.orig.z);
                s_item[11][k] = __float_as_uint(r_.pdfW);
                s_item[12][k] = __float_as_uint(r_.newDir.x); s_item[13][k] = __float_as_uint(r_.newDir.y); s_item[14][k] = __float_as_uint(r_.newDir.z);
                s_item[15][k] = sk;
            }
            __syncthreads();
            if (work) {
                o.bsdfNEE = mk3(__uint_as_float(s_item[0][slot]), __uint_as_float(s_item[1][slot]), __uint_as_float(s_item[2][slot]));
                o.bsdfPdfW = __uint_as_float(s_item[3][slot]); o.singular = s_item[4][slot];
                o.newT = mk3(__uint_as_float(s_item[5][slot]), __uint_as_float(s_item[6][slot]), __uint_as_float(s_item[7][slot]));
                o.orig = mk3(__uint_as_float(s_item[8][slot]), __uint_as_float(s_item[9][slot]), __uint_as_float(s_item[10][slot]));
                o.pdfW = __uint_as_float(s_item[11][slot]);
                o.newDir = mk3(__uint_as_float(s_item[12][slot]), __uint_as_float(s_item[13][slot]), __uint_as_float(s_item[14][slot]));
                seed = s_item[15][slot];
            }
        }
        if (!terminate && !regrouped) {
            if (inlined) {
                const f3 L = haveL ? Lnee : (FULL ? Lold : ld3(rd4(st.at(S_SHD, gid))));
                if (FUSE == USE_ALL) {
                    const float4 hp2 = rd4t(st.at(S_HITP, gid)), huv2 = rd4t(st.at(S_HITUV, gid)), d42 = rd4t(st.at(S_DIR, gid));
                    SurfHit h; h.P = ld3(hp2); h.N = hitN; h.uv = mk2(huv2.x, huv2.y);
                    o = material_step<FUSE>(sc, h, sc.materials[__float_as_int(huv2.w)], backface, ld3(d42), L, T, &seed);
                } else {
                    SurfHit h; h.P = hitP; h.N = hitN; h.uv = hitUV;
                    o = material_step<FUSE>(sc, h, mat, backface, rayDir, L, T, &seed);
                }
                if (!FULL) {
                    wr4(st.at(S_LBSDF, gid), mk4(o.bsdfNEE, o.bsdfPdfW));
                    wr4(st.at(S_LT, gid), mk4u(T, o.singular));
                    wr4(st.at(S_THR, gid), mk4u(o.newT, seed));
                    wr4(st.at(S_ORIG, gid), mk4(o.orig, o.pdfW));
                    wr4(st.at(S_DIR, gid), mk4u(o.newDir, len));
                }
            } else if (!FULL) {
                wr4(st.at(S_THR, gid), mk4u(T, seed));
                if (RAW && isRaw) wr4(st.at(S_DIR, gid), mk4u(rayDir, lenBits));
            }
        }
        if (FULL) {
            const bool c1 = !terminate && inlined, c0 = !terminate && !inlined && ml == 0u;
            float4 lbs = mk4(o.bsdfNEE, o.bsdfPdfW), lt4 = mk4u(T, o.singular), or4 = mk4(o.orig, o.pdfW), dr4 = mk4u(o.newDir, len);
            if (!c1) {
#ifdef FLX_LAB_LOGIC_NOOLD
                if (c0) lt4 = rd4(st.at(S_LT, gid));
#else
                if (terminate || c0) lt4 = rd4(st.at(S_LT, gid));
#endif
                if (!terminate) { dr4 = rd4t(st.at(S_DIR, gid)); dr4.w = __uint_as_float(lenBits); }
                if (c0) { lbs = rd4(st.at(S_LBSDF, gid)); or4 = rd4t(st.at(S_ORIG, gid)); }
            }
            float4 thr4 = mk4u(c1 ? o.newT : T, seed);
            if (regen && terminate) {
                uint32_t sd = seed; f3 ro, rd;
                camera_ray(fr, p, regenLocal, &sd, &ro, &rd);
                or4 = mk4(ro, 1.0f);
                dr4 = mk4u(rd, FLX_FRESH | 0u);
                thr4 = mk4u(mk3(1.0f), sd);
                st.firstDiffuse[gid] = 0u;
                if (aux.appendExt) qs.q[FLX_Q_EXTENSION][ext_len(qs) + regenRank] = gid;
            }
            if (prep && terminate) {
                uint32_t sd = seed;
                const float jx = rand01(&sd), jy = rand01(&sd);
                const uint32_t sd2 = sd;
                const f3 ro = camera_lens_origin(p, &sd);
                or4 = mk4(ro, 1.0f);
                dr4 = make_float4(jx, jy, __uint_as_float(sd2), __uint_as_float(FLX_FRESH | 0u));
                thr4 = mk4u(mk3(1.0f), sd);
            }
            st.blocked[gid] = (neeBlocked || ((regen || prep) && terminate)) ? 1u : blockedOld;
            wr4(st.at(S_LBSDF, gid), lbs);
            wr4(st.at(S_LT, gid), lt4);
            wr4(st.at(S_THR, gid), thr4);
            wr4(st.at(S_ORIG, gid), or4);
            wr4(st.at(S_DIR, gid), dr4);
            splat();
        }
    }

    if (gid < st.numTasks) aux.member[gid] = (uint8_t)member;

    __shared__ uint32_t s_cnt[NUM_LISTS][LOGIC_BLOCK / 64];
    const uint32_t wave = threadIdx.x >> 6;
    const uint32_t ml = member >> 2;
    uint64_t b0 = __ballot(member & 1u), b1 = __ballot(member & 2u);
    uint64_t m1 = __ballot(ml == 1u), m2 = __ballot(ml == 2u), m3 = __ballot(ml == 3u), m4 = __ballot(ml == 4u), m5 = __ballot(ml == 5u);
    if ((threadIdx.x & 63u) == 0u) {
        s_cnt[0][wave] = (uint32_t)__popcll(b0); s_cnt[1][wave] = (uint32_t)__popcll(b1);
        s_cnt[2][wave] = (uint32_t)__popcll(m1); s_cnt[3][wave] = (uint32_t)__popcll(m2);
        s_cnt[4][wave] = (uint32_t)__popcll(m3); s_cnt[5][wave] = (uint32_t)__popcll(m4); s_cnt[6][wave] = (uint32_t)__popcll(m5);
    }
    __syncthreads();
    if (threadIdx.x < NUM_LISTS) {
        uint32_t s = 0;
        for (int w = 0; w < LOGIC_BLOCK / 64; w++) s += s_cnt[threadIdx.x][w];
        aux.blockCounts[threadIdx.x * aux.stride + blockIdx.x] = s;
        if (s != 0u) atomicAdd(aux.segTotals + threadIdx.x * aux.numSegs + blockIdx.x / flxqb::QB_SEG_BLOCKS, s);
        if (blockIdx.x == 0u) aux.snapshot[threadIdx.x] = qs.counters[list_counter(threadIdx.x)];
    }
}

#ifndef QUEUE_BUILD_BLOCKS_PER_CU
#define QUEUE_BUILD_BLOCKS_PER_CU 4
#endif
struct QueueBuild {
    const uint8_t *member; const uint32_t *blockCounts; const uint32_t *totals; uint32_t *zero; const uint32_t *snapshot;
    uint32_t stride, numTasks, numSegs, totalsWords;
    uint32_t parts;
    int fuse; uint32_t raygenFirst, byPathId;
};
__device__ __forceinline__ uint32_t wave_sum(uint32_t v) { for (int d = 32; d > 0; d >>= 1) v += __shfl_xor(v, d, 64); return v; }
__device__ __forceinline__ uint32_t prefix_of_count4(uint32_t n) { return mbcnt(__ballot(n & 1u)) + 2u * mbcnt(__ballot(n & 2u)) + 4u * mbcnt(__ballot(n & 4u)); }
__device__ __forceinline__ void emit4(uint32_t *q, uint32_t slot, uint32_t bits, uint32_t gid)
{
    if (bits == 0xFu && (slot & 3u) == 0u) { *reinterpret_cast<uint4 *>(q + slot) = make_uint4(gid, gid + 1u, gid + 2u, gid + 3u); return; }
    if (bits & 1u) q[slot++] = gid;
    if (bits & 2u) q[slot++] = gid + 1u;
    if (bits & 4u) q[slot++] = gid + 2u;
    if (bits & 8u) q[slot] = gid + 3u;
}
__device__ __forceinline__ uint32_t load_member4(const uint8_t *member, uint64_t p, uint32_t numTasks)
{
    const uint32_t valid = flxqb::qb_valid(p, numTasks);
    if (valid == 4u) return *reinterpret_cast<const uint32_t *>(member + p);
    uint32_t w = 0u;
    for (uint32_t k = 0; k < valid; k++) w |= (uint32_t)member[p + k] << (8u * k);
    return w;
}

__global__ __launch_bounds__(flxqb::QB_THREADS) void k_queue_build(Queues qs, QueueBuild a)
{
    using namespace flxqb;
    __shared__ uint32_t s_base[NUM_LISTS];
    __shared__ uint32_t s_new[NUM_LISTS];
    __shared__ uint32_t s_off[NUM_LISTS][QB_SEG_BLOCKS];
    const uint32_t lane = threadIdx.x & 63u, wave = threadIdx.x >> 6;
    uint32_t seg0, seg1;
    qb_owned(blockIdx.x, gridDim.x, a.numSegs, a.parts, &seg0, &seg1);
    uint32_t tile0, steps;
    qb_tiles(blockIdx.x, a.parts, &tile0, &steps);
    for (uint32_t i = blockIdx.x * QB_THREADS + threadIdx.x; i < a.totalsWords; i += gridDim.x * QB_THREADS) a.zero[i] = 0u;
    for (uint32_t l = wave; l < NUM_LISTS; l += QB_WAVES) {
        uint32_t before, all;
        qb_partial(a.totals + (size_t)l * a.numSegs, a.numSegs, seg0, lane, 64u, &before, &all);
        before = wave_sum(before); all = wave_sum(all);
        if (lane == 0u) { const uint32_t snap = a.snapshot[l]; s_base[l] = snap + before; s_new[l] = snap + all; }
    }
    __syncthreads();
    if (blockIdx.x == 0u && threadIdx.x < NUM_LISTS) qs.counters[list_counter(threadIdx.x)] = s_new[threadIdx.x];
    if (seg0 == seg1) return;
    uint32_t extBase = qs.counters[FLX_Q_EXTENSION];
    if (qs.extPend) for (uint32_t l = 0; l < NUM_LISTS; l++) if (qs.extPend & (1u << list_counter(l))) extBase += s_new[l];
    if (a.byPathId != 2u && a.raygenFirst) extBase += s_new[0];
    uint32_t *const outq[NUM_LISTS] = {qs.q[FLX_Q_RAYGEN], qs.q[FLX_Q_SHADOW], qs.q[FLX_Q_DIFFUSE], qs.q[FLX_Q_GLOSSY], qs.q[FLX_Q_GGX_REFL], qs.q[FLX_Q_GGX_REFR], qs.q[FLX_Q_DELTA]};
    uint32_t *const ext = qs.q[FLX_Q_EXTENSION];

    for (uint32_t seg = seg0; seg < seg1; seg++) {
        uint32_t mw[QB_STEPS];
        #pragma unroll
        for (uint32_t i = 0; i < QB_STEPS; i++) mw[i] = i < steps ? load_member4(a.member, qb_first_path(seg, tile0 + wave + QB_WAVES * i, lane), a.numTasks) : 0u;
        if (seg != seg0) __syncthreads();
        for (uint32_t l = wave; l < NUM_LISTS; l += QB_WAVES) {
            const uint32_t c = a.blockCounts[(size_t)l * a.stride + (size_t)seg * QB_SEG_BLOCKS + lane];
            uint32_t inc = c;
            for (int d = 1; d < 64; d <<= 1) { const uint32_t v = __shfl_up(inc, d, 64); if (lane >= (uint32_t)d) inc += v; }
            const uint32_t base = s_base[l];
            s_off[l][lane] = base + inc - c;
            if (lane == 63u) s_base[l] = base + inc;
        }
        __syncthreads();
        #pragma unroll
        for (uint32_t i = 0; i < QB_STEPS; i++) {
            if (i >= steps) break;
            const uint32_t tile = tile0 + wave + QB_WAVES * i;
            const uint32_t w = mw[i];
            const uint32_t gid = (uint32_t)qb_first_path(seg, tile, lane);
            if (__ballot(w != 0u) == 0ull) continue;
            uint32_t matOff = 0u;
            #pragma unroll
            for (int l = 0; l < NUM_LISTS; l++) {
                const uint32_t off = s_off[l][tile];
                if (l >= 2) matOff += off;
                const uint32_t bits = qb_bits(w, (uint32_t)l);
                if (__ballot(bits != 0u) == 0ull) continue;
                const uint32_t r = off + prefix_of_count4(qb_count4(bits));
                emit4(outq[l], r, bits, gid);
                if (a.fuse != 0 && a.byPathId == 0u && l >= 2 && fuse_inlines_list(a.fuse, (uint32_t)(l - 1))) {
                    uint32_t segBase = extBase;
                    for (int m = 2; m < l; m++) segBase += s_new[m];
                    emit4(ext, segBase + r, bits, gid);
                }
            }
            if (a.fuse != 0 && a.byPathId == 1u) {
                const uint32_t bits = qb_bits_material(w);
                emit4(ext, extBase + matOff + prefix_of_count4(qb_count4(bits)), bits, gid);
            }
            if (a.fuse != 0 && a.byPathId == 2u) {
                const uint32_t bits = qb_bits_traced(w);
                emit4(ext, extBase + s_off[0][tile] + matOff + prefix_of_count4(qb_count4(bits)), bits, gid);
            }
        }
    }
}

uint32_t logic_aux_stride(uint32_t numTasks) { return flxqb::qb_count_stride(numTasks); }
uint32_t logic_queue_aux_words(uint32_t numTasks) { return flxqb::qb_aux_words(numTasks); }

uint32_t fused_queue_mask(int fuse)
{
    uint32_t m = 0;
    for (uint32_t ml = 1; ml <= 5; ml++) if (fuse_inlines_list(fuse, ml)) m |= 1u << (FLX_Q_DIFFUSE + ml - 1);
    return m;
}

void launch_logic(hipStream_t s, const State &st, const Queues &qs, const Scene &sc, const Frame &fr, const flx_render_params &p,
                  uint8_t *member, uint32_t *blockCounts, uint32_t *queueAux, int firstIteration, int fuse, int raygenFirst, int extByPathId, int raw,
                  unsigned long long *lookback, uint32_t epoch, int regen, int regenAppendExt, uint32_t *error, int regroup, uint32_t parity, uint32_t numCUs,
                  const MeshLights *meshLights)
{
    uint32_t blocks = (st.numTasks + LOGIC_BLOCK - 1) / LOGIC_BLOCK;
    const uint32_t tw = flxqb::qb_totals_words(st.numTasks);
    parity &= 1u;
    uint32_t *const totals = queueAux + (size_t)parity * tw;
    LogicAux aux{member, blockCounts, totals, queueAux + flxqb::qb_snapshot_at(st.numTasks), blocks, flxqb::qb_segments(st.numTasks), logic_aux_stride(st.numTasks),
                 lookback, epoch, (uint32_t)(raw ? regen : 0), (uint32_t)regenAppendExt, error};
    const bool rg = LOGIC_REGROUP && raw && regroup && fuse == USE_ALL && !firstIteration && st.numTasks % LOGIC_BLOCK == 0u;
    const dim3 g(blocks), b(LOGIC_BLOCK);
    switch (fuse) {
    case USE_DIFFUSE:
        if (raw) hipLaunchKernelGGL((k_logic<USE_DIFFUSE, true>), g, b, 0, s, st, sc, fr, p, aux, qs, (uint32_t)firstIteration, MeshArg<false>());
        else hipLaunchKernelGGL((k_logic<USE_DIFFUSE, false>), g, b, 0, s, st, sc, fr, p, aux, qs, (uint32_t)firstIteration, MeshArg<false>());
        break;
    case USE_ALL:
        if (rg) hipLaunchKernelGGL((k_logic<USE_ALL, true, true>), g, b, 0, s, st, sc, fr, p, aux, qs, (uint32_t)firstIteration, MeshArg<false>());
        else if (raw) hipLaunchKernelGGL((k_logic<USE_ALL, true>), g, b, 0, s, st, sc, fr, p, aux, qs, (uint32_t)firstIteration, MeshArg<false>());
        else hipLaunchKernelGGL((k_logic<USE_ALL, false>), g, b, 0, s, st, sc, fr, p, aux, qs, (uint32_t)firstIteration, MeshArg<false>());
        break;
    default:
        fuse = 0;
        if (meshLights) hipLaunchKernelGGL((k_logic<0, false, false, true>), g, b, 0, s, st, sc, fr, p, aux, qs, (uint32_t)firstIteration, MeshArg<true>{*meshLights});
        else hipLaunchKernelGGL(k_logic<0>, g, b, 0, s, st, sc, fr, p, aux, qs, (uint32_t)firstIteration, MeshArg<false>());
        break;
    }
    const QueueBuild qb{member, blockCounts, totals, queueAux + (size_t)(parity ^ 1u) * tw, aux.snapshot, aux.stride, st.numTasks, aux.numSegs, tw, flxqb::qb_parts(aux.numSegs, numCUs, QUEUE_BUILD_BLOCKS_PER_CU), fuse, (uint32_t)raygenFirst, (uint32_t)extByPathId};
    hipLaunchKernelGGL(k_queue_build, dim3(flxqb::qb_grid(aux.numSegs, numCUs, QUEUE_BUILD_BLOCKS_PER_CU)), dim3(flxqb::QB_THREADS), 0, s, qs, qb);
}
int logic_can_regenerate() { return LOGIC_FULL_STORES != 0 ? 1 : 0; }
uint32_t logic_lookback_words(uint32_t numTasks) { return (numTasks + 63u) / 64u; }

}
```

fluctus_amd/csrc/material.hip:

```cpp
#include "flx_bsdf.h"
#include "flx_launch.h"

namespace flxd {

#ifndef MAT_BLOCK
#define MAT_BLOCK 64
#endif

#define FLX_NO_APPEND 0x80000000u
template <int USE>
__device__ __forceinline__ void material_body(const State &st, const Queues &qs, const Scene &sc, int queueId, uint32_t idx, uint32_t earlierMask)
{
    const uint32_t qlen = qs.counters[queueId];
    const bool active = idx < qlen;
    uint32_t gid = 0;
    if (active) {
        gid = qs.q[queueId][idx];
        const float4 thr = rd4t(st.at(S_THR, gid));
        const float4 hp = rd4t(st.at(S_HITP, gid));
        const float4 hn = rd4t(st.at(S_HITN, gid));
        const float4 huv = rd4t(st.at(S_HITUV, gid));
        const float4 d4 = rd4t(st.at(S_DIR, gid));
        const float4 sd = rd4t(st.at(S_SHD, gid));
        uint32_t seed = __float_as_uint(thr.w);
        SurfHit h; h.P = ld3(hp); h.N = ld3(hn); h.uv = mk2(huv.x, huv.y);
        const bool backface = (__float_as_uint(hn.w) & 2u) != 0u;
        const f3 oldT = ld3(thr);
        const MatStep o = material_step<USE>(sc, h, sc.materials[__float_as_int(huv.w)], backface, ld3(d4), ld3(sd), oldT, &seed);

        wr4(st.at(S_LBSDF, gid), mk4(o.bsdfNEE, o.bsdfPdfW));
        wr4(st.at(S_LT, gid), mk4u(oldT, o.singular));
        wr4(st.at(S_THR, gid), mk4u(o.newT, seed));
        wr4(st.at(S_ORIG, gid), mk4(o.orig, o.pdfW));
        wr4(st.at(S_DIR, gid), mk4u(o.newDir, __float_as_uint(d4.w) & ~FLX_FRESH));
    }
    if (active && !(earlierMask & FLX_NO_APPEND)) {
        uint32_t base = ext_len(qs);
        for (int q = FLX_Q_DIFFUSE; q < FLX_NUM_QUEUES; q++) if (earlierMask & (1u << q)) base += qs.counters[q];
        qs.q[FLX_Q_EXTENSION][base + idx] = gid;
    }
}

#define MAT_GRID 4096u
template <int USE>
__global__ __launch_bounds__(MAT_BLOCK) void k_material(State st, Queues qs, Scene sc, int queueId, uint32_t earlierMask)
{
    const uint32_t nb = (qs.counters[queueId] + MAT_BLOCK - 1) / MAT_BLOCK;
    for (uint32_t b = blockIdx.x; b < nb; b += gridDim.x)
        material_body<USE>(st, qs, sc, queueId, b * MAT_BLOCK + threadIdx.x, earlierMask);
}

__global__ __launch_bounds__(MAT_BLOCK) void k_material_rest(State st, Queues qs, Scene sc, uint32_t doneMask)
{
    const uint32_t noAppend = doneMask & FLX_NO_APPEND;
    uint32_t nbq[4], total = 0;
    for (int q = FLX_Q_GLOSSY; q <= FLX_Q_DELTA; q++) {
        nbq[q - FLX_Q_GLOSSY] = (doneMask & (1u << q)) ? 0u : (qs.counters[q] + MAT_BLOCK - 1) / MAT_BLOCK;
        total += nbq[q - FLX_Q_GLOSSY];
    }
    for (uint32_t vb = blockIdx.x; vb < total; vb += gridDim.x) {
        uint32_t b = vb;
        uint32_t earlier = (1u << FLX_Q_DIFFUSE) | noAppend;
        for (int q = FLX_Q_GLOSSY; q <= FLX_Q_DELTA; q++) {
            const uint32_t nb = nbq[q - FLX_Q_GLOSSY];
            if (b < nb) { material_body<USE_GLOSSY | USE_GGX_REFL | USE_GGX_REFR | USE_DELTA>(st, qs, sc, q, b * MAT_BLOCK + threadIdx.x, earlier); break; }
            b -= nb;
            earlier |= 1u << q;
        }
    }
}

void launch_bump_extension(hipStream_t s, uint32_t *counters, uint32_t srcMask);

static void launch_one(hipStream_t s, const State &st, const Queues &qs, const Scene &sc, int queueId, int use, uint32_t earlierMask)
{
    uint32_t blocks = (st.numTasks + MAT_BLOCK - 1) / MAT_BLOCK;
    if (blocks > MAT_GRID) blocks = MAT_GRID;
    switch (use) {
    case USE_DIFFUSE: hipLaunchKernelGGL(k_material<USE_DIFFUSE>, dim3(blocks), dim3(MAT_BLOCK), 0, s, st, qs, sc, queueId, earlierMask); break;
    case USE_GLOSSY: hipLaunchKernelGGL(k_material<USE_GLOSSY>, dim3(blocks), dim3(MAT_BLOCK), 0, s, st, qs, sc, queueId, earlierMask); break;
    case USE_GGX_REFL: hipLaunchKernelGGL(k_material<USE_GGX_REFL>, dim3(blocks), dim3(MAT_BLOCK), 0, s, st, qs, sc, queueId, earlierMask); break;
    case USE_GGX_REFR: hipLaunchKernelGGL(k_material<USE_GGX_REFR>, dim3(blocks), dim3(MAT_BLOCK), 0, s, st, qs, sc, queueId, earlierMask); break;
    case USE_DELTA: hipLaunchKernelGGL(k_material<USE_DELTA>, dim3(blocks), dim3(MAT_BLOCK), 0, s, st, qs, sc, queueId, earlierMask); break;
    default: hipLaunchKernelGGL(k_material<USE_ALL>, dim3(blocks), dim3(MAT_BLOCK), 0, s, st, qs, sc, queueId, earlierMask); break;
    }
}

void launch_materials(hipStream_t s, const State &st, const Queues &qs, const Scene &sc, uint32_t separateQueues)
{
    if (separateQueues) {
        const uint32_t D = 1u << FLX_Q_DIFFUSE, G = 1u << FLX_Q_GLOSSY, RL = 1u << FLX_Q_GGX_REFL, RR = 1u << FLX_Q_GGX_REFR, DL = 1u << FLX_Q_DELTA;
        launch_one(s, st, qs, sc, FLX_Q_DIFFUSE, USE_DIFFUSE, 0u);
        {
            uint32_t blocks = (st.numTasks + MAT_BLOCK - 1) / MAT_BLOCK + 4;
            if (blocks > MAT_GRID) blocks = MAT_GRID;
            hipLaunchKernelGGL(k_material_rest, dim3(blocks), dim3(MAT_BLOCK), 0, s, st, qs, sc, 0u);
        }
        (void)G; (void)RL; (void)RR; (void)DL; (void)D;
    } else {
        launch_one(s, st, qs, sc, FLX_Q_DIFFUSE, USE_ALL, 0u);
    }
}

void launch_materials_after_fused(hipStream_t s, const State &st, const Queues &qs, const Scene &sc, uint32_t doneMask, int extWritten)
{
    const uint32_t FLX_NO_APPEND_ = extWritten ? FLX_NO_APPEND : 0u;
    const uint32_t all = (1u << FLX_Q_DIFFUSE) | (1u << FLX_Q_GLOSSY) | (1u << FLX_Q_GGX_REFL) | (1u << FLX_Q_GGX_REFR) | (1u << FLX_Q_DELTA);
    if ((doneMask & all) == all) return;
    if (!(doneMask & (1u << FLX_Q_DIFFUSE))) launch_one(s, st, qs, sc, FLX_Q_DIFFUSE, USE_DIFFUSE, FLX_NO_APPEND_);
    if ((doneMask & (all & ~(1u << FLX_Q_DIFFUSE))) != (all & ~(1u << FLX_Q_DIFFUSE))) {
        uint32_t blocks = (st.numTasks + MAT_BLOCK - 1) / MAT_BLOCK + 4;
        if (blocks > MAT_GRID) blocks = MAT_GRID;
        hipLaunchKernelGGL(k_material_rest, dim3(blocks), dim3(MAT_BLOCK), 0, s, st, qs, sc, doneMask | FLX_NO_APPEND_);
    }
}

}
```

fluctus_amd/csrc/trace4r.hip:

```cpp
#include "flx_trace4.h"
#include <cstdlib>
#include "flx_launch.h"

namespace flxd {

#ifndef WIDE_R_MIN_WAVES
#define WIDE_R_MIN_WAVES 1
#endif
#define R_NONE 0xFFFFFFFFu

#ifdef FLX_LAB_RSTATS
unsigned long long *g_lab_rstats = nullptr;
#define RSTAT(k, v) do { if (ANY_HIT == false && rstats) { acc[k] += (unsigned long long)(v); } } while (0)
#else
#define RSTAT(k, v) do { } while (0)
#endif

template <bool ANY_HIT, int ANY_ORDER>
__global__ __launch_bounds__(WIDE_BLOCK, WIDE_R_MIN_WAVES) void k_trace4r(State st, Queues qs, Scene sc, flx_render_params p, TraceAux aux, int refillMin, int waitMax, uint32_t *cursor)
{
    __shared__ uint32_t s_stack[WIDE_LDS_LEVELS * WIDE_BLOCK];
#ifdef FLX_LAB_RSTATS
    unsigned long long *rstats = aux.stats; unsigned long long acc[6] = {0, 0, 0, 0, 0, 0};
#endif
    const int QID = ANY_HIT ? FLX_Q_SHADOW : FLX_Q_EXTENSION;
    const uint32_t qlen = ANY_HIT ? qs.counters[QID] : ext_len(qs);
    const uint32_t *queue = qs.q[QID];
    const uint32_t nblk = (qlen + 63u) >> 6;
    uint32_t xcdList = blockIdx.x & 7u, listsTried = 0;
    auto issue_fetch = [&]() -> uint32_t {
        uint32_t k = 0;
        if (threadIdx.x == 0) k = atomicAdd(&cursor[xcdList * FLX_CURSOR_STRIDE], 1u);
        return k;
    };
    auto resolve = [&](uint32_t ticket) -> uint32_t {
        for (;;) {
            const uint32_t b = (uint32_t)__builtin_amdgcn_readfirstlane((int)ticket) * 8u + xcdList;
            if (b < nblk) return b;
            if (++listsTried >= 8u) return 0xFFFFFFFFu;
            xcdList = (xcdList + 1u) & 7u;
            ticket = issue_fetch();
        }
    };
    uint32_t blk = resolve(issue_fetch()), pos = 0;
    if (blk >= nblk) return;
    uint32_t nextTicket = issue_fetch();
    uint32_t gidBlk = queue[min((blk << 6) + threadIdx.x, qlen - 1u)];

    WStack stk;
    stk.lds = s_stack + threadIdx.x;
    stk.stride = aux.totalThreads;
    stk.spill = aux.spill + (blockIdx.x * WIDE_BLOCK + threadIdx.x);
    stk.base = 0;
    const float4 *wn = reinterpret_cast<const float4 *>(sc.wnodes);

    WRay r; r.setup(mk3(0.0f), mk3(1.0f), sc.wideClamp);
    uint32_t gid = R_NONE, cur = FLX_RAY_DONE;
    int sp = 0;
    float tbest = 0.0f, ubest = 0.0f, vbest = 0.0f;
    int tribest = -1;
    bool occluded = false;
    uint32_t nT = 0;

    for (;;) {
        const bool idle = cur == FLX_RAY_DONE;
        const uint64_t idleMask = __ballot(idle);
        const uint32_t nIdle = (uint32_t)__popcll(idleMask);
        if ((int)nIdle >= refillMin || nIdle == 64u) {
            if (idle && gid != R_NONE) {
                if (ANY_HIT) st.blocked[gid] = occluded ? 1u : 0u;
                else wr4(st.at(S_HITUV, gid), make_float4(ubest, vbest, __uint_as_float(FLX_RAW | (uint32_t)(tribest + 1)), tbest));
                gid = R_NONE;
            }
            if (blk < nblk) {
                const uint32_t blkLen = min(64u, qlen - (blk << 6));
                const uint32_t avail = blkLen - pos;
                const uint32_t rank = mbcnt(idleMask);
                const uint32_t cand = (uint32_t)__shfl((int)gidBlk, (int)((pos + rank) & 63u), 64);
                if (idle && rank < avail) {
                    gid = cand;
                    const float4 o4 = rd4(st.at(ANY_HIT ? S_SHO : S_ORIG, gid));
                    const float4 d4 = rd4(st.at(ANY_HIT ? S_SHD : S_DIR, gid));
                    r.setup(ld3(o4), ld3(d4), sc.wideClamp);
                    tbest = ANY_HIT ? o4.w : FLX_FLT_MAX;
                    ubest = 0.0f; vbest = 0.0f; tribest = -1; occluded = false;
                    sp = 0; stk.base = 0; cur = sc.wrootRef;
                }
                pos += min(nIdle, avail);
                if (pos >= blkLen) {
                    blk = resolve(nextTicket); pos = 0;
                    if (blk < nblk) { nextTicket = issue_fetch(); gidBlk = queue[min((blk << 6) + threadIdx.x, qlen - 1u)]; }
                }
            } else if (nIdle == 64u) break;
        }
        for (;;) {
            const bool inner = !(cur & FLX_WIDE_LEAF_BIT);
            const uint64_t mI = __ballot(inner);
            if (mI == 0ull) break;
            const int nDone = (int)__popcll(__ballot(cur == FLX_RAY_DONE));
            if (64 - (int)__popcll(mI) - nDone >= waitMax) break;
            if (blk < nblk && nDone >= refillMin && waitMax < 64) break;
            RSTAT(0, 1); RSTAT(1, __popcll(mI));
            if (inner) wide_node_visit<ANY_HIT, ANY_ORDER>(wn, stk, r, tbest, sp, cur);
        }
#ifdef FLX_LAB_RSTATS
        { const uint64_t mL = __ballot(cur != FLX_RAY_DONE && (cur & FLX_WIDE_LEAF_BIT)); if (mL) { RSTAT(2, 1); RSTAT(3, __popcll(mL)); } }
#endif
        if (cur != FLX_RAY_DONE && (cur & FLX_WIDE_LEAF_BIT)) {
#ifdef FLX_LAB_RSTATS
            {
                const float4 *lp = sc.wleaf + (cur & FLX_WIDE_OFF_MASK);
                const float4 b0 = lp[0], b1 = lp[1];
                const float bmin[3] = {b0.x, b0.y, b0.z}, bmax[3] = {b1.x, b1.y, b1.z};
                float tnear;
                bool hitAny = false;
                if (slab(bmin, bmax, r.orig, r.dinv, tbest, &tnear)) {
                    const int count = __float_as_int(b0.w);
                    const float4 *tp = lp + 2;
                    for (int k = 0; k < count; k++, tp += 3) {
                        if (ANY_HIT == false && rstats) { const uint64_t m_ = __ballot(true); if (lane_id() == (uint32_t)__ffsll((long long)m_) - 1u) { atomicAdd(&rstats[22], 1ull); atomicAdd(&rstats[23], (unsigned long long)__popcll(m_)); } }
                        float t, u, v;
                        const float4 a = tp[0], b = tp[1], c = tp[2];
                        if (moller_trumbore(r.orig, r.dir, ld3(a), ld3(b), ld3(c), &t, &u, &v) && t > 0.0f && t < tbest) {
                            if (ANY_HIT) { hitAny = true; break; }
                            tbest = t; ubest = u; vbest = v; tribest = __float_as_int(a.w);
                        }
                    }
                }
                if (hitAny) { occluded = true; cur = FLX_RAY_DONE; } else cur = stk.pop(sp);
            }
#else
            if (wide_leaf_visit<ANY_HIT, false>(sc.wleaf, r, cur, tbest, ubest, vbest, tribest, nT, nullptr)) { occluded = true; cur = FLX_RAY_DONE; }
            else cur = stk.pop(sp);
#endif
        }
    }
#ifdef FLX_LAB_RSTATS
    if (ANY_HIT == false && rstats && threadIdx.x == 0) for (int k = 0; k < 4; k++) atomicAdd(&rstats[18 + k], acc[k]);
#endif
}

__global__ __launch_bounds__(256) void k_materialise(State st, Scene sc, flx_render_params p)
{
    for (uint32_t gid = blockIdx.x * blockDim.x + threadIdx.x; gid < st.numTasks; gid += gridDim.x * blockDim.x) {
        const float4 raw = rd4t(st.at(S_HITUV, gid));
        if (!hit_is_raw(__float_as_uint(raw.z))) continue;
        const float4 o4 = rd4(st.at(S_ORIG, gid));
        const float4 d4 = rd4(st.at(S_DIR, gid));
        const f3 orig = ld3(o4), dir = ld3(d4);
        const HitVals h = hit_values_raw(sc, p, orig, dir, raw);
        wr4(st.at(S_DIR, gid), mk4u(dir, __float_as_uint(d4.w) + 1u));
        wr4(st.at(S_HITP, gid), mk4(h.P, h.t));
        const uint32_t keep = hit_keep_flags(d4.w, __float_as_uint(reinterpret_cast<const float *>(st.at(S_HITN, gid))[3]));
        wr4(st.at(S_HITN, gid), mk4u(h.N, h.flags | keep));
        wr4(st.at(S_HITUV, gid), make_float4(h.tu, h.tv, __int_as_float(h.tri), __int_as_float(h.matId)));
    }
}

__global__ __launch_bounds__(256) void k_lightfix4(State st, Queues qs, flx_render_params p)
{
    const uint32_t qlen = qs.counters[FLX_Q_SHADOW];
    for (uint32_t idx = blockIdx.x * blockDim.x + threadIdx.x; idx < qlen; idx += gridDim.x * blockDim.x) {
        const uint32_t gid = qs.q[FLX_Q_SHADOW][idx];
        if (st.blocked[gid]) continue;
        const float4 o4 = rd4(st.at(S_SHO, gid)), d4 = rd4(st.at(S_SHD, gid));
        float tl = o4.w;
        if (light_quad(p.areaLight, ld3(o4), ld3(d4), &tl)) st.blocked[gid] = 1u;
    }
}

template <class K>
static uint32_t persistent_grid(K kernel, int &cached, uint32_t numCUs, uint32_t numTasks, const char *capEnv = nullptr)
{
    if (cached == 0) {
        int n = 0;
        if (hipOccupancyMaxActiveBlocksPerMultiprocessor(&n, reinterpret_cast<const void *>(kernel), WIDE_BLOCK, 0) != hipSuccess || n <= 0) n = 16;
        cached = n;
    }
    int perCU = cached;
#ifdef FLX_LAB
    { static const char *e = getenv("FLX_PERSISTENT_WAVES_PER_CU"); if (e && atoi(e) > 0 && atoi(e) < perCU) perCU = atoi(e); }
    if (capEnv) { const char *e = getenv(capEnv); if (e && atoi(e) > 0 && atoi(e) < perCU) perCU = atoi(e); }
#else
    (void)capEnv;
#endif
    uint32_t g = numCUs * (uint32_t)perCU;
    const uint32_t blocks = (numTasks + 63u) / 64u;
    if (blocks / 3u < g) g = blocks / 3u > numCUs ? blocks / 3u : numCUs;
    return g < blocks ? g : blocks;
}

void launch_extend4r(hipStream_t s, const State &st, const Queues &qs, const Scene &sc, const flx_render_params &p, uint32_t *spill, uint32_t numCUs, int refill, uint32_t *cursor)
{
    const int refillMin = (refill & 0xFF) ? (refill & 0xFF) : 1, waitMax = ((refill >> 8) & 0xFF) ? ((refill >> 8) & 0xFF) : 64;
    static int occ = 0;
    TraceAux aux{spill, ((st.numTasks + 255u) / 256u) * 256u, nullptr};
#ifdef FLX_LAB_RSTATS
    aux.stats = g_lab_rstats;
#endif
    const uint32_t grid = persistent_grid(k_trace4r<false, 0>, occ, numCUs, st.numTasks, "FLX_PERSISTENT_WAVES_EXT");
    hipLaunchKernelGGL((k_trace4r<false, 0>), dim3(grid), dim3(WIDE_BLOCK), 0, s, st, qs, sc, p, aux, refillMin, waitMax, cursor);
}

void launch_materialise(hipStream_t s, const State &st, const Scene &sc, const flx_render_params &p, uint32_t numCUs)
{
    hipLaunchKernelGGL(k_materialise, dim3(numCUs * 8), dim3(256), 0, s, st, sc, p);
}

void launch_shadow4r(hipStream_t s, const State &st, const Queues &qs, const Scene &sc, const flx_render_params &p, uint32_t *spill, uint32_t numCUs, int refill, uint32_t *cursor)
{
    const int refillMin = (refill & 0xFF) ? (refill & 0xFF) : 1, waitMax = ((refill >> 8) & 0xFF) ? ((refill >> 8) & 0xFF) : 64;
    static int occ[2] = {0, 0};
    TraceAux aux{spill, ((st.numTasks + 255u) / 256u) * 256u, nullptr};
    if (p.useEnvMap && !p.useAreaLight) {
        const uint32_t grid = persistent_grid(k_trace4r<true, 1>, occ[1], numCUs, st.numTasks, "FLX_PERSISTENT_WAVES_SHADOW");
        hipLaunchKernelGGL((k_trace4r<true, 1>), dim3(grid), dim3(WIDE_BLOCK), 0, s, st, qs, sc, p, aux, refillMin, waitMax, cursor);
    } else {
        const uint32_t grid = persistent_grid(k_trace4r<true, 0>, occ[0], numCUs, st.numTasks, "FLX_PERSISTENT_WAVES_SHADOW");
        hipLaunchKernelGGL((k_trace4r<true, 0>), dim3(grid), dim3(WIDE_BLOCK), 0, s, st, qs, sc, p, aux, refillMin, waitMax, cursor);
    }
    if (p.useAreaLight) hipLaunchKernelGGL(k_lightfix4, dim3(numCUs * 8), dim3(256), 0, s, st, qs, p);
}

}
```

Measured before the change: 6893 Mrays/s.

## Defer committing raw hit records in fused diffuse logic, settle lazily

Adds a lazy hit-commit mode for the raw-hit fused-diffuse logic kernel. The kernel skips writing HITP/HITUV for paths that continue into non-diffuse material queues, and writes the new ray origin and direction into double-buffered arrays that are swapped on the host. Non-diffuse material kernels reconstruct the surface hit from the raw record on demand, and a settle kernel commits any remaining raw hits only when another stage needs them. The goal is to cut global-memory stores in the logic pass, at the cost of extra state buffers, recomputing hits in material kernels, and more complex phase bookkeeping.

```diff
diff --git a/fluctus_amd/csrc/api.hip b/fluctus_amd/csrc/api.hip
--- a/fluctus_amd/csrc/api.hip
+++ b/fluctus_amd/csrc/api.hip
@@ -117,6 +117,10 @@
     for (int r = 0; r < S_NUM_REC; r++) {
         if (dalloc(c, c->fixedAllocs, &c->st.rec[r], N)) return fail("hipMalloc(state)", hipErrorOutOfMemory);
         (void)hipMemsetAsync(c->st.rec[r], 0, N * sizeof(float4), c->stream);
+    }
+    for (int r = 0; r < 2; r++) {
+        if (dalloc(c, c->fixedAllocs, &c->st.other[r], N)) return fail("hipMalloc(state)", hipErrorOutOfMemory);
+        (void)hipMemsetAsync(c->st.other[r], 0, N * sizeof(float4), c->stream);
     }
     if (dalloc(c, c->fixedAllocs, &c->st.phase, N) || dalloc(c, c->fixedAllocs, &c->mkStats, 4)) return fail("hipMalloc(state)", hipErrorOutOfMemory);
     (void)hipMemsetAsync(c->st.phase, 0, N * 4, c->stream); (void)hipMemsetAsync(c->mkStats, 0, 16, c->stream);
@@ -332,6 +336,7 @@
     if (name && strcmp(name, "ext_order") == 0 && value >= 0 && value <= 2) { c->extOrder = value; return 0; }
     if (name && strcmp(name, "regen") == 0 && (value == 0 || value == 1)) { if (value && optionBuffers(c, false, true)) return 1; c->regenOpt = value; return 0; }
     if (name && strcmp(name, "regen_prep") == 0 && (value == 0 || value == 1)) { c->prepOpt = value; return 0; }
+    if (name && strcmp(name, "lazy_hit_commit") == 0 && (value == 0 || value == 1)) { c->lazyCommitOpt = value; return 0; }
     if (name && strcmp(name, "regroup") == 0 && value >= -1 && value <= 1) { c->regroupOpt = value; c->regroup = value >= 0 ? value : c->regroupAuto; return 0; }
     if (name && strcmp(name, "fuse_set") == 0 && (value == 1 || value == 31)) { c->fuseSet = value; return 0; }
     if (name && strcmp(name, "overlap") == 0 && value >= -1 && value <= 2) { ENTER(c, CALL_OBSERVE); c->overlapOpt = value; pickSchedule(c); return 0; }
@@ -384,14 +389,14 @@
 }
 static int phaseCode(const flx_ctx *c)
 {
-    return c->phase | (c->rawHits ? 8 : 0) | (c->matQueuesEmpty ? 16 : 0);
+    return c->phase | (c->rawHits ? 8 : 0) | (c->matQueuesEmpty ? 16 : 0) | (c->prevHitsPending ? 32 : 0);
 }
 int flx_get_option(flx_ctx *c, const char *name, int *value)
 {
     NEED(c, name && value, "flx_get_option: null");
     const struct { const char *n; int v; } tab[] = {
         {"xcd_remap", c->xcdRemap}, {"fuse", c->fuse}, {"overlap", c->overlap}, {"shadow_tree", c->shadowTree}, {"extend_tree", c->extendTree},
-        {"denoiser", c->denoiser}, {"moments", c->moments}, {"motion_history", c->motionHistory}, {"deform_history", c->deformHistory},{"mesh_lights", c->ml.state.on ? 1 : 0}, {"mesh_lights_wavefront", c->ml.state.wavefront ? 1 : 0}, {"eager_bump", c->eagerBump}, {"node_layout", c->nodeLayout}, {"fuse_set", c->fuseSet}, {"ext_order", c->extOrder}, {"regen", c->regenOpt}, {"regroup", c->regroup}, {"regen_prep", c->prepOpt}, {"refill_extend", c->refillExt}, {"refill_shadow", c->refillShadow}, {"shadow_split", c->shadowSplit}, {"fused_queue_mask", (int)fused_queue_mask(fuseSetNow(c))}, {"fuse_set_now", fuseSetNow(c)}};
+        {"denoiser", c->denoiser}, {"moments", c->moments}, {"motion_history", c->motionHistory}, {"deform_history", c->deformHistory},{"mesh_lights", c->ml.state.on ? 1 : 0}, {"mesh_lights_wavefront", c->ml.state.wavefront ? 1 : 0}, {"eager_bump", c->eagerBump}, {"node_layout", c->nodeLayout}, {"fuse_set", c->fuseSet}, {"ext_order", c->extOrder}, {"regen", c->regenOpt}, {"regroup", c->regroup}, {"regen_prep", c->prepOpt}, {"lazy_hit_commit", c->lazyCommitOpt}, {"refill_extend", c->refillExt}, {"refill_shadow", c->refillShadow}, {"shadow_split", c->shadowSplit}, {"fused_queue_mask", (int)fused_queue_mask(fuseSetNow(c))}, {"fuse_set_now", fuseSetNow(c)}};
     for (const auto &t : tab) if (strcmp(name, t.n) == 0) { *value = t.v; return 0; }
     if (strcmp(name, "phase") == 0) { *value = phaseCode(c); return 0; }
     if (strcmp(name, "wide_far") == 0) { *value = wideFar(c); return 0; }
diff --git a/fluctus_amd/csrc/api_wavefront.hip b/fluctus_amd/csrc/api_wavefront.hip
--- a/fluctus_amd/csrc/api_wavefront.hip
+++ b/fluctus_amd/csrc/api_wavefront.hip
@@ -1,24 +1,24 @@
 #include "flx_ctx.h"
 
-struct Step { bool launchDeferred, commitRaw; int next; };
+struct Step { bool launchDeferred, commitRaw, settlePrev; int next; };
 static Step transition(int ph, Call call)
 {
     const bool deferred = ph == PH_DEFER_LOGIC || ph == PH_DEFER_LOGIC_RAYGEN;
     const bool chain = deferred || ph == PH_CHAIN || ph == PH_CHAIN_EXT;
     switch (call) {
-    case CALL_LOGIC:     return {deferred, false, PH_IDLE};
-    case CALL_RAYGEN:    if (ph == PH_DEFER_LOGIC) return {false, false, PH_DEFER_LOGIC_RAYGEN};
-                         return {deferred, false, chain ? PH_CHAIN : PH_IDLE};
-    case CALL_MATERIALS: if (deferred) return {false, false, PH_CHAIN};
-                         return {false, true, chain ? PH_CHAIN : PH_IDLE};
-    case CALL_EXTEND:    return {deferred, true, chain ? PH_CHAIN_EXT : PH_EXT};
-    case CALL_SHADOW:    return {deferred, false, PH_IDLE};
-    case CALL_QUIET:     return {deferred, false, deferred ? PH_CHAIN : ph};
-    case CALL_NEUTRAL:   return {deferred, false, PH_IDLE};
-    case CALL_PEEK:      return {deferred, true, deferred ? PH_CHAIN : ph};
-    case CALL_OBSERVE:   return {deferred, true, PH_IDLE};
-    }
-    return {deferred, true, PH_IDLE};
+    case CALL_LOGIC:     return {deferred, false, true, PH_IDLE};
+    case CALL_RAYGEN:    if (ph == PH_DEFER_LOGIC) return {false, false, false, PH_DEFER_LOGIC_RAYGEN};
+                         return {deferred, false, false, chain ? PH_CHAIN : PH_IDLE};
+    case CALL_MATERIALS: if (deferred) return {false, false, false, PH_CHAIN};
+                         return {false, true, true, chain ? PH_CHAIN : PH_IDLE};
+    case CALL_EXTEND:    return {deferred, true, ph != PH_CHAIN, chain ? PH_CHAIN_EXT : PH_EXT};
+    case CALL_SHADOW:    return {deferred, false, false, PH_IDLE};
+    case CALL_QUIET:     return {deferred, false, false, deferred ? PH_CHAIN : ph};
+    case CALL_NEUTRAL:   return {deferred, false, false, PH_IDLE};
+    case CALL_PEEK:      return {deferred, true, true, deferred ? PH_CHAIN : ph};
+    case CALL_OBSERVE:   return {deferred, true, true, PH_IDLE};
+    }
+    return {deferred, true, true, PH_IDLE};
 }
 void flxd::flushExt(flx_ctx *c) { if (c->qs.extPend) { launch_bump_extension(c->stream, c->qs.counters, c->qs.extPend); c->qs.extPend = 0; } }
 static void flushExtIfPending(flx_ctx *c, uint32_t bits) { if (c->qs.extPend & bits) flushExt(c); }
@@ -40,11 +40,21 @@
     LAUNCHED(c);
     return 0;
 }
+static int settlePrevHits(flx_ctx *c)
+{
+    if (!c->prevHitsPending) return 0;
+    c->prevHitsPending = false;
+    HIPCHK(c, hipSetDevice(c->device));
+    launch_settle_hits(c->stream, c->st, c->sc, c->params, (uint32_t)c->numCUs);
+    LAUNCHED(c);
+    return 0;
+}
 static int extOrderFor(const flx_ctx *c, int fused, int raygenFirst) { return !fused ? 0 : (c->extOrder == 2 && (!raygenFirst || !c->raygenQueueEmpty)) ? 1 : c->extOrder; }
 int flxd::fuseSetNow(const flx_ctx *c) { return c->params.wfSeparateQueues ? c->fuseSet : 31; }
 static int runLogic(flx_ctx *c, int first, int fused, int raygenFirst)
 {
     const int raw = (c->rawHits && fused != 0 && raygenFirst && !first) ? 1 : 0;
+    if (settlePrevHits(c)) return 1;
     if (!raw && materialise(c)) return 1;
     c->rawHits = false;
     flushExt(c);
@@ -57,12 +67,14 @@
     if (regen) c->regenUsed = true;
     const int prep = (raw && !regen && c->prepOpt && c->raygenQueueEmpty && c->fr.localPixels > 0) ? 1 : 0;
     c->prepDone = prep != 0;
+    const int lazy = (raw && c->lazyCommitOpt && logic_can_lazy_commit(fused)) ? 1 : 0;
     if (++c->logicEpoch == 0u) c->logicEpoch = 1u;
-    { ScopedTimer t(c, fused ? FLX_K_LOGIC_FUSED : FLX_K_LOGIC); launch_logic(c->stream, c->st, c->qs, c->sc, c->fr, c->params, c->member, c->blockCounts, c->queueAux, first, fused, raygenFirst, order, raw,
+    { ScopedTimer t(c, fused ? FLX_K_LOGIC_FUSED : FLX_K_LOGIC); launch_logic(c->stream, c->st, c->qs, c->sc, c->fr, c->params, c->member, c->blockCounts, c->queueAux, first, fused, raygenFirst, order, raw, lazy,
                                                                                 c->lookback, c->logicEpoch, regen ? 1 : (prep ? 2 : 0), order == 2 ? 0 : 1, c->logicError, c->regroup,
                                                                                 c->queueParity ^= 1u, (uint32_t)c->numCUs,
                                                                                 (!fused && c->ml.state.litWavefront()) ? &c->ml.t : nullptr); }
     LAUNCHED(c);
+    if (lazy) { std::swap(c->st.rec[S_ORIG], c->st.other[0]); std::swap(c->st.rec[S_DIR], c->st.other[1]); c->prevHitsPending = true; }
     c->matQueuesEmpty = false; c->raygenQueueEmpty = false;
     if (c->overlap == 2) HIPCHK(c, hipEventRecord(c->evPostLogic, c->stream));
     return 0;
@@ -81,6 +93,7 @@
         if (runLogic(c, c->pendFirst, 0, 0)) return 1;
         if (withRaygen && runRaygen(c)) return 1;
     }
+    if (st.settlePrev && settlePrevHits(c)) return 1;
     if (st.commitRaw && materialise(c)) return 1;
     c->phase = st.next;
     return 0;
@@ -99,6 +112,7 @@
 {
     READY(c, CALL_EXTEND);
     const bool chainIntact = c->phase == PH_CHAIN_EXT;
+    c->prevHitsPending = false;
     if (c->overlap && !(c->overlap == 2 && chainIntact)) HIPCHK(c, hipEventRecord(c->evPreExt, c->stream));
     if (c->profile == 1 || c->profile == 2) { if (c->spanStart) c->eventPool.push_back(c->spanStart); c->spanStart = getEvent(c); (void)hipEventRecord(c->spanStart, c->stream); }
     {
diff --git a/fluctus_amd/csrc/flx_ctx.h b/fluctus_amd/csrc/flx_ctx.h
--- a/fluctus_amd/csrc/flx_ctx.h
+++ b/fluctus_amd/csrc/flx_ctx.h
@@ -70,6 +70,8 @@
     uint32_t splitLimit = 0;
     uint32_t *splitCounts = nullptr; uint4 *splitRecA = nullptr, *splitRecB = nullptr; uint32_t splitCapA = 0, splitCapB = 0;
     bool rawHits = false;
+    bool prevHitsPending = false;
+    int lazyCommitOpt = 1;
     bool cursorDirty[2] = {false, false};
 
     uint32_t wideInfo[8] = {0, 0, 0, 0, 0, 0, 0, 0};
diff --git a/fluctus_amd/csrc/flx_device.h b/fluctus_amd/csrc/flx_device.h
--- a/fluctus_amd/csrc/flx_device.h
+++ b/fluctus_amd/csrc/flx_device.h
@@ -13,6 +13,7 @@
 struct State {
     float4 *rec[S_NUM_REC];
     __host__ __device__ __forceinline__ float4 *at(int r, uint32_t gid) const { return rec[r] + (size_t)gid; }
+    float4 *other[2];
     uint32_t *blocked;
     float *pickProb;
     uint32_t *firstDiffuse;
diff --git a/fluctus_amd/csrc/flx_launch.h b/fluctus_amd/csrc/flx_launch.h
--- a/fluctus_amd/csrc/flx_launch.h
+++ b/fluctus_amd/csrc/flx_launch.h
@@ -66,12 +66,14 @@
 uint32_t shadow_split_lists(); uint32_t shadow_split_count_words();
 void launch_extend4r(hipStream_t, const State &, const Queues &, const Scene &, const flx_render_params &, uint32_t *, uint32_t, int, uint32_t *);
 void launch_shadow4r(hipStream_t, const State &, const Queues &, const Scene &, const flx_render_params &, uint32_t *, uint32_t, int, uint32_t *);
-void launch_logic(hipStream_t, const State &, const Queues &, const Scene &, const Frame &, const flx_render_params &, uint8_t *, uint32_t *, uint32_t *, int, int, int, int, int,
+void launch_logic(hipStream_t, const State &, const Queues &, const Scene &, const Frame &, const flx_render_params &, uint8_t *, uint32_t *, uint32_t *, int, int, int, int, int, int,
                   unsigned long long *, uint32_t, int, int, uint32_t *, int, uint32_t, uint32_t, const MeshLights *);
 void launch_env_nee_table(hipStream_t, const Scene &, float4 *, uint32_t);
 int logic_can_regenerate();
+int logic_can_lazy_commit(int fuse);
 uint32_t logic_lookback_words(uint32_t numTasks);
 void launch_materialise(hipStream_t, const State &, const Scene &, const flx_render_params &, uint32_t);
+void launch_settle_hits(hipStream_t, const State &, const Scene &, const flx_render_params &, uint32_t);
 void launch_materials(hipStream_t, const State &, const Queues &, const Scene &, uint32_t);
 void launch_materials_after_fused(hipStream_t, const State &, const Queues &, const Scene &, uint32_t, int);
 uint32_t fused_queue_mask(int);
diff --git a/fluctus_amd/csrc/flx_trace.h b/fluctus_amd/csrc/flx_trace.h
--- a/fluctus_amd/csrc/flx_trace.h
+++ b/fluctus_amd/csrc/flx_trace.h
@@ -127,6 +127,11 @@
 __device__ __forceinline__ HitVals hit_values_raw(const Scene &sc, const flx_render_params &p, f3 orig, f3 dir, float4 raw)
 {
     return hit_values<true>(sc, p, orig, dir, raw.w, raw.x, raw.y, (int)(__float_as_uint(raw.z) & FLX_RAW_TRI) - 1);
+}
+__device__ __forceinline__ HitVals hit_surface_raw(const Scene &sc, f3 orig, f3 dir, float4 raw)
+{
+    const flx_render_params none{};
+    return hit_values<false>(sc, none, orig, dir, raw.w, raw.x, raw.y, (int)(__float_as_uint(raw.z) & FLX_RAW_TRI) - 1);
 }
 
 struct Stack {
diff --git a/fluctus_amd/csrc/logic.hip b/fluctus_amd/csrc/logic.hip
--- a/fluctus_amd/csrc/logic.hip
+++ b/fluctus_amd/csrc/logic.hip
@@ -108,7 +108,7 @@
 #ifndef LOGIC_MIN_BLOCKS
 #define LOGIC_MIN_BLOCKS 0
 #endif
-template <int FUSE, bool RAW = false, bool REGROUP = false, bool MESH = false>
+template <int FUSE, bool RAW = false, bool REGROUP = false, bool MESH = false, bool LAZY = false>
 __global__ __launch_bounds__(LOGIC_BLOCK, (REGROUP ? LOGIC_REGROUP_MIN_BLOCKS : LOGIC_MIN_BLOCKS) > 0 ? (REGROUP ? LOGIC_REGROUP_MIN_BLOCKS : LOGIC_MIN_BLOCKS) : 1) void k_logic(State st, Scene sc, Frame fr, flx_render_params p, LogicAux aux, Queues qs, uint32_t firstIteration, MeshArg<MESH> meshArg)
 {
     const MeshLights mesh = meshArg.get();
@@ -210,6 +210,7 @@
         }
 
         constexpr bool FULL = LOGIC_FULL_STORES != 0 && RAW && FUSE != 0;
+        static_assert(!LAZY || (FULL && FUSE != USE_ALL && !REGROUP), "the lazy commit is a variant of the full-store pass that keeps its hit record in registers");
         uint32_t regenRank = 0u, regenLocal = 0u;
         const bool regen = FULL && aux.regen == 1u;
         const bool prep = FULL && aux.regen == 2u;
@@ -355,7 +356,7 @@
             }
             const float4 hp4 = mk4(hitP, hitT), huv4 = make_float4(hitUV.x, hitUV.y, __int_as_float(hitI), __int_as_float(hitMat));
             if (FUSE == USE_ALL) { wr4t(st.at(S_HITP, gid), hp4); wr4t(st.at(S_HITUV, gid), huv4); }
-            else { wr4(st.at(S_HITP, gid), hp4); wr4(st.at(S_HITUV, gid), huv4); }
+            else if (!LAZY || (!terminate && ml == 0u)) { wr4(st.at(S_HITP, gid), hp4); wr4(st.at(S_HITUV, gid), huv4); }
             wr4(st.at(S_HITN, gid), mk4u(hitN, (hflags & 1u) | (backface ? 2u : 0u)));
             wr4(st.at(S_SHO, gid), sho);
             wr4(st.at(S_SHD, gid), shd);
@@ -487,8 +488,8 @@
             wr4(st.at(S_LBSDF, gid), lbs);
             wr4(st.at(S_LT, gid), lt4);
             wr4(st.at(S_THR, gid), thr4);
-            wr4(st.at(S_ORIG, gid), or4);
-            wr4(st.at(S_DIR, gid), dr4);
+            wr4((LAZY ? st.other[0] : st.rec[S_ORIG]) + (size_t)gid, or4);
+            wr4((LAZY ? st.other[1] : st.rec[S_DIR]) + (size_t)gid, dr4);
             splat();
         }
     }
@@ -629,7 +630,7 @@
 }
 
 void launch_logic(hipStream_t s, const State &st, const Queues &qs, const Scene &sc, const Frame &fr, const flx_render_params &p,
-                  uint8_t *member, uint32_t *blockCounts, uint32_t *queueAux, int firstIteration, int fuse, int raygenFirst, int extByPathId, int raw,
+                  uint8_t *member, uint32_t *blockCounts, uint32_t *queueAux, int firstIteration, int fuse, int raygenFirst, int extByPathId, int raw, int lazyCommit,
                   unsigned long long *lookback, uint32_t epoch, int regen, int regenAppendExt, uint32_t *error, int regroup, uint32_t parity, uint32_t numCUs,
                   const MeshLights *meshLights)
 {
@@ -643,7 +644,8 @@
     const dim3 g(blocks), b(LOGIC_BLOCK);
     switch (fuse) {
     case USE_DIFFUSE:
-        if (raw) hipLaunchKernelGGL((k_logic<USE_DIFFUSE, true>), g, b, 0, s, st, sc, fr, p, aux, qs, (uint32_t)firstIteration, MeshArg<false>());
+        if (raw && lazyCommit && logic_can_lazy_commit(fuse)) hipLaunchKernelGGL((k_logic<USE_DIFFUSE, true, false, false, true>), g, b, 0, s, st, sc, fr, p, aux, qs, (uint32_t)firstIteration, MeshArg<false>());
+        else if (raw) hipLaunchKernelGGL((k_logic<USE_DIFFUSE, true>), g, b, 0, s, st, sc, fr, p, aux, qs, (uint32_t)firstIteration, MeshArg<false>());
         else hipLaunchKernelGGL((k_logic<USE_DIFFUSE, false>), g, b, 0, s, st, sc, fr, p, aux, qs, (uint32_t)firstIteration, MeshArg<false>());
         break;
     case USE_ALL:
@@ -661,6 +663,7 @@
     hipLaunchKernelGGL(k_queue_build, dim3(flxqb::qb_grid(aux.numSegs, numCUs, QUEUE_BUILD_BLOCKS_PER_CU)), dim3(flxqb::QB_THREADS), 0, s, qs, qb);
 }
 int logic_can_regenerate() { return LOGIC_FULL_STORES != 0 ? 1 : 0; }
+int logic_can_lazy_commit(int fuse) { return (LOGIC_FULL_STORES != 0 && fuse == USE_DIFFUSE) ? 1 : 0; }
 uint32_t logic_lookback_words(uint32_t numTasks) { return (numTasks + 63u) / 64u; }
 
 }
diff --git a/fluctus_amd/csrc/material.hip b/fluctus_amd/csrc/material.hip
--- a/fluctus_amd/csrc/material.hip
+++ b/fluctus_amd/csrc/material.hip
@@ -1,4 +1,5 @@
 #include "flx_bsdf.h"
+#include "flx_trace.h"
 #include "flx_launch.h"
 
 namespace flxd {
@@ -8,7 +9,7 @@
 #endif
 
 #define FLX_NO_APPEND 0x80000000u
-template <int USE>
+template <int USE, bool LAZY = false>
 __device__ __forceinline__ void material_body(const State &st, const Queues &qs, const Scene &sc, int queueId, uint32_t idx, uint32_t earlierMask)
 {
     const uint32_t qlen = qs.counters[queueId];
@@ -24,9 +25,16 @@
         const float4 sd = rd4t(st.at(S_SHD, gid));
         uint32_t seed = __float_as_uint(thr.w);
         SurfHit h; h.P = ld3(hp); h.N = ld3(hn); h.uv = mk2(huv.x, huv.y);
+        int matId = __float_as_int(huv.w);
+        if constexpr (LAZY) {
+            if (hit_is_raw(__float_as_uint(huv.z))) {
+                const HitVals hv = hit_surface_raw(sc, ld3(rd4(st.other[0] + (size_t)gid)), ld3(d4), huv);
+                h.P = hv.P; h.uv = mk2(hv.tu, hv.tv); matId = hv.matId;
+            }
+        }
         const bool backface = (__float_as_uint(hn.w) & 2u) != 0u;
         const f3 oldT = ld3(thr);
-        const MatStep o = material_step<USE>(sc, h, sc.materials[__float_as_int(huv.w)], backface, ld3(d4), ld3(sd), oldT, &seed);
+        const MatStep o = material_step<USE>(sc, h, sc.materials[matId], backface, ld3(d4), ld3(sd), oldT, &seed);
 
         wr4(st.at(S_LBSDF, gid), mk4(o.bsdfNEE, o.bsdfPdfW));
         wr4(st.at(S_LT, gid), mk4u(oldT, o.singular));
@@ -50,6 +58,7 @@
         material_body<USE>(st, qs, sc, queueId, b * MAT_BLOCK + threadIdx.x, earlierMask);
 }
 
+template <bool LAZY>
 __global__ __launch_bounds__(MAT_BLOCK) void k_material_rest(State st, Queues qs, Scene sc, uint32_t doneMask)
 {
     const uint32_t noAppend = doneMask & FLX_NO_APPEND;
@@ -63,7 +72,7 @@
         uint32_t earlier = (1u << FLX_Q_DIFFUSE) | noAppend;
         for (int q = FLX_Q_GLOSSY; q <= FLX_Q_DELTA; q++) {
             const uint32_t nb = nbq[q - FLX_Q_GLOSSY];
-            if (b < nb) { material_body<USE_GLOSSY | USE_GGX_REFL | USE_GGX_REFR | USE_DELTA>(st, qs, sc, q, b * MAT_BLOCK + threadIdx.x, earlier); break; }
+            if (b < nb) { material_body<USE_GLOSSY | USE_GGX_REFL | USE_GGX_REFR | USE_DELTA, LAZY>(st, qs, sc, q, b * MAT_BLOCK + threadIdx.x, earlier); break; }
             b -= nb;
             earlier |= 1u << q;
         }
@@ -94,7 +103,7 @@
         {
             uint32_t blocks = (st.numTasks + MAT_BLOCK - 1) / MAT_BLOCK + 4;
             if (blocks > MAT_GRID) blocks = MAT_GRID;
-            hipLaunchKernelGGL(k_material_rest, dim3(blocks), dim3(MAT_BLOCK), 0, s, st, qs, sc, 0u);
+            hipLaunchKernelGGL(k_material_rest<false>, dim3(blocks), dim3(MAT_BLOCK), 0, s, st, qs, sc, 0u);
         }
         (void)G; (void)RL; (void)RR; (void)DL; (void)D;
     } else {
@@ -111,7 +120,7 @@
     if ((doneMask & (all & ~(1u << FLX_Q_DIFFUSE))) != (all & ~(1u << FLX_Q_DIFFUSE))) {
         uint32_t blocks = (st.numTasks + MAT_BLOCK - 1) / MAT_BLOCK + 4;
         if (blocks > MAT_GRID) blocks = MAT_GRID;
-        hipLaunchKernelGGL(k_material_rest, dim3(blocks), dim3(MAT_BLOCK), 0, s, st, qs, sc, doneMask | FLX_NO_APPEND_);
+        hipLaunchKernelGGL(k_material_rest<true>, dim3(blocks), dim3(MAT_BLOCK), 0, s, st, qs, sc, doneMask | FLX_NO_APPEND_);
     }
 }
 
diff --git a/fluctus_amd/csrc/trace4r.hip b/fluctus_amd/csrc/trace4r.hip
--- a/fluctus_amd/csrc/trace4r.hip
+++ b/fluctus_amd/csrc/trace4r.hip
@@ -157,6 +157,19 @@
     }
 }
 
+__global__ __launch_bounds__(256) void k_settle_hits(State st, Scene sc, flx_render_params p)
+{
+    for (uint32_t gid = blockIdx.x * blockDim.x + threadIdx.x; gid < st.numTasks; gid += gridDim.x * blockDim.x) {
+        const float4 raw = rd4t(st.at(S_HITUV, gid));
+        if (!hit_is_raw(__float_as_uint(raw.z))) continue;
+        const float4 o4 = rd4(st.other[0] + (size_t)gid);
+        const float4 d4 = rd4(st.other[1] + (size_t)gid);
+        const HitVals h = hit_values_raw(sc, p, ld3(o4), ld3(d4), raw);
+        wr4(st.at(S_HITP, gid), mk4(h.P, h.t));
+        wr4(st.at(S_HITUV, gid), make_float4(h.tu, h.tv, __int_as_float(h.tri), __int_as_float(h.matId)));
+    }
+}
+
 __global__ __launch_bounds__(256) void k_lightfix4(State st, Queues qs, flx_render_params p)
 {
     const uint32_t qlen = qs.counters[FLX_Q_SHADOW];
@@ -207,7 +220,12 @@
     hipLaunchKernelGGL(k_materialise, dim3(numCUs * 8), dim3(256), 0, s, st, sc, p);
 }
 
-void launch_shadow4r(hipStream_t s, const State &st, const Queues &qs, const Scene &sc, const flx_render_params &p, uint32_t *spill, uint32_t numCUs, int refill, uint32_t *cursor)
+void launch_settle_hits(hipStream_t s, const State &st, const Scene &sc, const flx_render_params &p, uint32_t numCUs)
+{
+    hipLaunchKernelGGL(k_settle_hits, dim3(numCUs * 8), dim3(256), 0, s, st, sc, p);
+}
+
+void launch_shadow4r(hipStream_t s,const State &st, const Queues &qs, const Scene &sc, const flx_render_params &p, uint32_t *spill, uint32_t numCUs, int refill, uint32_t *cursor)
 {
     const int refillMin = (refill & 0xFF) ? (refill & 0xFF) : 1, waitMax = ((refill >> 8) & 0xFF) ? ((refill >> 8) & 0xFF) : 64;
     static int occ[2] = {0, 0};
```

Measured after the change: 7073 Mrays/s, median of 6. 2.6% higher.
